# Aseeef/seq-align-gpu

Hardware: AMD Instinct MI355X
Metric: GCUPS (DP cell updates/s) at 1/2/4/8 MI355X; bit-exact max scores vs CPU ref (higher is better)
Workload: dtype f16

## Files before the change

seq-align-gpu_amd/__init__.py:

```python
import ctypes as C
import os

import numpy as np

_HERE = os.path.dirname(os.path.abspath(__file__))
LIB_PATH = os.path.join(_HERE, "libswg.so")
DATA_DIR = os.path.join(_HERE, "data")
CLI_PATH = os.path.join(_HERE, "bin", "smith_waterman")

if not os.path.exists(LIB_PATH):
    raise ImportError(
        "libswg.so is not built: run `python seq-align-gpu_amd/build.py` "
        "(or __graft_entry__.build()); there is no Python/CPU fallback")

lib = C.CDLL(LIB_PATH, mode=C.RTLD_GLOBAL)

SWG_OK, SWG_ERR_ARG, SWG_ERR_HIP, SWG_ERR_NOMEM = 0, -1, -2, -3
SWG_ERR_STATE, SWG_ERR_RESIDUE, SWG_ERR_IO, SWG_ERR_NODEVICE = -4, -5, -6, -7

ABI_SYMBOLS = [
    "swg_create", "swg_destroy", "swg_last_error", "swg_global_error", "swg_abi_version", "swg_prune_last",
    "swg_set_option", "swg_set_scoring", "swg_set_query", "swg_set_query_pssm", "swg_db_pack", "swg_db_pack_shard", "swg_db_pack_shards", "swg_db_upload", "swg_db_view",
    "swg_db_free", "swg_db_save", "swg_db_load", "swg_db_count", "swg_db_total_count", "swg_db_residues",
    "swg_db_packed_bytes", "swg_db_order", "swg_search", "swg_search_begin", "swg_search_end", "swg_search_multi",
# ... 187 lines not shown
_sig("swg_group_create", C.c_int, [_vp, C.c_int, C.c_int, C.POINTER(_vp)])
_sig("swg_group_destroy", None, [_vp])
_sig("swg_group_size", C.c_int, [_vp])
_sig("swg_group_last_error", C.c_char_p, [_vp])
_sig("swg_group_set_option", C.c_int, [_vp, C.c_char_p, C.c_long])
_sig("swg_group_set_scoring", C.c_int, [_vp, _vp, C.c_int, C.c_int])
_sig("swg_group_set_query", C.c_int, [_vp, _vp, C.c_size_t])
_sig("swg_group_set_query_pssm", C.c_int, [_vp, _vp, C.c_size_t])
_sig("swg_group_load", C.c_int, [_vp, _vp, _vp, C.c_size_t])
_sig("swg_group_search", C.c_int, [_vp, _vp, _vp, C.c_size_t, C.POINTER(C.c_size_t), C.POINTER(Stats)])
_sig("swg_letter_index", C.c_int, [C.c_int])
_sig("swg_index_letter", C.c_int, [C.c_int])
_sig("swg_scoring_init", None, [C.POINTER(Scoring)])
_sig("swg_scoring_add", C.c_int, [C.POINTER(Scoring), C.c_int, C.c_int, C.c_int])
_sig("swg_scoring_load_matrix", C.c_int, [C.POINTER(Scoring), C.c_char_p, C.c_char_p, C.c_size_t])
_sig("swg_query_sanitize", None, [C.POINTER(Scoring), _vp, C.c_size_t])
_sig("swg_seqs_read", C.c_int, [C.c_char_p, C.c_size_t, C.POINTER(Seqs), C.c_char_p, C.c_size_t])
_sig("swg_seqs_free", None, [C.POINTER(Seqs)])
_sig("swg_seqs_to_indices", C.c_int, [C.POINTER(Seqs), _vp, C.c_char_p])
_sig("swg_synth_db", C.c_int, [C.c_uint64, C.c_size_t, C.c_double, C.c_double, C.c_uint32,
                               C.c_uint32, C.POINTER(_vp), C.POINTER(_vp)])
_sig("swg_synth_query", None, [C.c_uint64, C.c_size_t, _vp])
_sig("swg_synth_db_similar", C.c_int, [C.c_uint64, C.c_size_t, C.c_double, C.c_double, C.c_uint32,
                                       C.c_uint32, _vp, C.c_size_t, C.c_double, C.c_double,
                                       C.POINTER(_vp), C.POINTER(_vp), C.POINTER(C.c_size_t)])
_sig("swg_synth_db_family", C.c_int, [C.c_uint64, C.c_size_t, C.c_double, C.c_double, C.c_uint32,
                                      C.c_uint32, _vp, C.c_size_t, C.c_double, C.c_double, C.c_double,
                                      C.POINTER(_vp), C.POINTER(_vp), C.POINTER(C.c_size_t)])
_sig("swg_synth_db_shard", C.c_int, [C.c_uint64, C.c_size_t, C.c_double, C.c_double, C.c_uint32, C.c_uint32,
                                     _vp, C.c_size_t, C.c_double, C.c_double, C.c_int, C.c_int,
                                     C.POINTER(_vp), C.POINTER(_vp), C.POINTER(_vp), C.POINTER(C.c_size_t),
                                     C.POINTER(C.c_uint64), C.POINTER(C.c_size_t)])
_sig("swg_synth_free", None, [_vp])
_sig("swg_pssm_load", C.c_int, [C.c_char_p, C.POINTER(Scoring), C.POINTER(_vp), C.POINTER(_vp), C.POINTER(C.c_size_t),
                                C.c_char_p, C.c_size_t])
_sig("swg_pssm_free", None, [_vp, _vp])
_sig("swg_debug_fail_alloc", None, [C.c_int])
_sig("swg_align_stats", C.c_int, [_vp, _vp, _vp, C.c_size_t, _vp, _vp])
_sig("swg_align_stats_multi", C.c_int, [_vp, _vp, _vp, _vp, C.c_size_t, _vp, C.c_size_t, _vp, _vp, _vp])
_sig("swg_align_stats_multi_pssm", C.c_int, [_vp, _vp, _vp, _vp, C.c_size_t, _vp, C.c_size_t, _vp, _vp, _vp])
_sig("swg_debug_bounds_last", C.c_int, [_vp, _vp])
_sig("swg_debug_sort_count", C.c_ulong, [])
_sig("swg_debug_engine", C.c_int, [_vp, C.c_size_t, C.c_int, C.c_int, _vp])
_sig("swg_debug_plan", C.c_int, [_vp, C.c_size_t, C.c_int, _vp])
_sig("swg_debug_plan_f16", C.c_int, [_vp, C.c_size_t, C.c_int, C.c_long, _vp])
_sig("swg_debug_plan_gapless", C.c_int, [_vp, C.c_size_t, C.c_int, _vp])
_sig("swg_debug_plan_forced", C.c_int, [_vp, C.c_size_t, C.c_int, C.c_long, C.c_long, C.c_long, C.c_int, C.c_long, C.c_int, _vp])
_sig("swg_debug_plan_streams", C.c_int, [_vp, _vp, _vp, C.c_size_t, C.c_int, C.c_long, C.c_long, C.c_long, C.c_long, _vp])
_sig("swg_debug_plan_systolic", C.c_int, [_vp, _vp, _vp, C.c_size_t, C.c_int, C.c_int, C.c_int, C.c_long, C.c_long, C.c_long, C.c_long, C.c_long, _vp])
_sig("swg_debug_systolic_variants", C.c_int, [C.c_int, _vp, C.c_size_t])
_sig("swg_debug_plan_batch", C.c_int, [_vp, C.c_size_t, C.c_size_t, C.c_int, C.c_int, C.c_int, C.c_long, C.c_long, C.c_long, _vp])
_sig("swg_debug_plan_lists", C.c_int, [_vp, C.c_size_t, C.c_size_t, C.c_int, C.c_int, C.c_long, C.c_long, C.c_long, _vp])
_sig("swg_debug_launch_log", None, [C.c_int])
_sig("swg_debug_launch_log_read", C.c_size_t, [_vp, C.c_size_t])
_sig("swg_debug_split", C.c_int, [_vp, C.c_size_t, C.c_uint64, _vp])
_sig("swg_debug_list_plan", C.c_int, [C.c_size_t, C.c_uint32, C.c_int, _vp, _vp])
_sig("swg_debug_pair_tokens", C.c_int, [_vp, _vp, C.c_int, _vp, C.c_size_t, C.POINTER(C.c_size_t)])
_sig("swg_debug_view_ranks", C.c_int, [_vp, _vp, C.c_size_t, _vp, C.POINTER(C.c_size_t)])
_sig("swg_debug_list_jobs", C.c_int, [_vp, _vp, _vp, C.c_size_t, _vp, C.c_size_t, C.POINTER(C.c_size_t), _vp])
_sig("swg_prune_last", C.c_int, [_vp, _vp])
_sig("swg_debug_prune_bound", C.c_int, [_vp, _vp, C.c_size_t, _vp, _vp, C.c_size_t, _vp, _vp])
_sig("swg_debug_prune_plan", C.c_int, [_vp, _vp])
_sig("swg_debug_prune_plan_above", C.c_int, [_vp, _vp])
_sig("swg_debug_above_multi_route", C.c_int, [C.c_long, C.c_int, C.c_int])
_sig("swg_debug_prune_stages", C.c_int, [_vp, _vp, C.c_size_t, C.POINTER(C.c_size_t)])
_sig("swg_debug_prune_kmer", C.c_int, [_vp, _vp, C.c_size_t, C.c_int, C.c_int, C.c_int, _vp, _vp, C.c_size_t, _vp, _vp])
_sig("swg_debug_prune_kmer_choice", C.c_int, [_vp, _vp])
_sig("swg_debug_prune_kmer_read", C.c_int, [_vp, _vp, C.c_int, _vp, _vp, C.c_size_t, _vp])
_sig("swg_debug_prune_kmer_seg", C.c_int, [_vp, _vp, C.c_size_t, C.c_int, C.c_int, C.c_int, C.c_int, _vp, _vp, C.c_size_t, _vp, _vp])
_sig("swg_debug_prune_kmer_choice_seg", C.c_int, [_vp, _vp])
_sig("swg_debug_prune_kmer_seg_read", C.c_int, [_vp, _vp, C.c_int, C.c_int, _vp, _vp, C.c_size_t, _vp])
_sig("swg_debug_prune_kmer_refine", C.c_int, [_vp, _vp, C.c_size_t, C.c_int, C.c_int, C.c_int, _vp, _vp, C.c_size_t, _vp, _vp])
_sig("swg_debug_prune_refine_choice", C.c_int, [_vp, _vp])
_sig("swg_debug_prune_refine_read", C.c_int, [_vp, _vp, C.c_int, _vp, _vp, _vp, C.c_size_t, _vp, C.c_size_t, _vp])
_sig("swg_debug_prune_stages3", C.c_int, [_vp, _vp, C.c_size_t, C.POINTER(C.c_size_t)])
_sig("swg_debug_prune_kmer_refine3", C.c_int, [_vp, _vp, C.c_size_t, C.c_int, C.c_int, C.c_int, _vp, _vp, C.c_size_t, _vp, _vp])
_sig("swg_debug_prune_refine3_choice", C.c_int, [_vp, _vp])
_sig("swg_debug_prune_kmer_refine4", C.c_int, [_vp, _vp, C.c_size_t, C.c_int, C.c_int, C.c_int, _vp, _vp, C.c_size_t, _vp])
_sig("swg_debug_prune_table_bits", C.c_int, [_vp, _vp, C.c_size_t, C.c_int])
_sig("swg_debug_prune_tables", C.c_int, [_vp, _vp])
_sig("swg_debug_prune_tables4", C.c_int, [_vp, _vp])
_sig("swg_debug_prune_refine4_read", C.c_int, [_vp, _vp, C.c_size_t, _vp])
_sig("swg_debug_prune_refine4_choice", C.c_int, [_vp, _vp])
_sig("swg_debug_prune_stages4", C.c_int, [_vp, _vp, C.c_size_t, C.POINTER(C.c_size_t)])
_sig("swg_debug_list_deal", C.c_int, [_vp, _vp, _vp, C.c_size_t, C.c_uint64, C.c_uint64, _vp, C.c_size_t, C.POINTER(C.c_size_t)])
_sig("swg_debug_calib_iters", C.c_int, [_vp, _vp, C.c_size_t, C.POINTER(C.c_size_t)])
_sig("swg_db_composition", C.c_int, [_vp, _vp, _vp])
_sig("swg_calibrate", C.c_int, [_vp, _vp, C.c_int, _vp])
_sig("swg_calibrate_multi", C.c_int, [_vp, _vp, _vp, C.c_size_t, _vp, C.c_int, _vp])
_sig("swg_calibrate_multi_pssm", C.c_int, [_vp, _vp, _vp, C.c_size_t, _vp, C.c_int, _vp])
_sig("swg_evalue", C.c_double, [_vp, C.c_uint64, C.c_int32])
_sig("swg_bitscore", C.c_double, [_vp, C.c_int32])
_sig("swg_evalue_min_score", C.c_int32, [_vp, C.c_uint64, C.c_double])
_sig("swg_synth_db_iid", C.c_int, [C.c_uint64, C.c_size_t, C.c_uint32, _vp, C.POINTER(_vp), C.POINTER(_vp)])
_sig("swg_gumbel_fit_hist", C.c_int, [_vp, C.c_size_t, C.POINTER(C.c_double), C.POINTER(C.c_double), C.POINTER(C.c_int)])
_sig("swg_matrix_lambda", C.c_int, [_vp, _vp, C.POINTER(C.c_double)])
_sig("swg_pssm_from_paths", C.c_int, [_vp, _vp, C.c_double, _vp, C.c_size_t, _vp, _vp, _vp, _vp, C.c_size_t, C.c_size_t, _vp, _vp, _vp])
_sig("swg_pssm_save", C.c_int, [C.c_char_p, _vp, _vp, C.c_size_t])
_sig("swg_pssm_build", C.c_int, [_vp, _vp, _vp, C.c_size_t, _vp, _vp, C.c_double, _vp, _vp, _vp])
_sig("swg_pssm_build_multi", C.c_int, [_vp, _vp, _vp, _vp, C.c_size_t, _vp, C.c_size_t, _vp, _vp, C.c_double, _vp, _vp, _vp])
_sig("swg_pssm_build_multi_pssm", C.c_int, [_vp, _vp, _vp, _vp, _vp, C.c_size_t, _vp, C.c_size_t, _vp, _vp, C.c_double, _vp, _vp, _vp])
_sig("swg_mask_params_default", None, [_vp])
_sig("swg_mask_tables", C.c_int, [_vp, _vp, C.POINTER(C.c_int64), C.POINTER(C.c_int64)])
_sig("swg_seg_mask", C.c_int, [_vp, C.c_size_t, _vp, _vp, C.POINTER(C.c_size_t)])
_sig("swg_seg_mask_segments", C.c_int, [_vp, C.c_size_t, _vp, _vp, C.POINTER(C.c_size_t), C.POINTER(C.c_size_t)])
_sig("swg_seg_mask_flat", C.c_int, [_vp, _vp, C.c_size_t, _vp, _vp])
_sig("swg_db_sequence", C.c_int, [_vp, C.c_uint32, _vp, C.c_size_t, C.POINTER(C.c_size_t)])
_sig("swg_db_mask", C.c_int, [_vp, _vp, _vp, C.POINTER(_vp)])
_sig("swg_db_mask_info", C.c_int, [_vp, _vp])
_sig("swg_debug_mask_fail_alloc", None, [C.c_int])


def _check(rc, ctx=None):
    if rc != SWG_OK:
        msg = lib.swg_last_error(ctx) if ctx else lib.swg_global_error()
        raise SwgError(rc, (msg or b"").decode("utf-8", "replace"))


def _i8(a):
    a = np.ascontiguousarray(a, dtype=np.int8)
    return a, a.ctypes.data_as(_vp)


def _pssm(pssm):
    a = np.asarray(pssm)
    if a.ndim != 2 or a.shape[1] != 32:
        raise ValueError("a PSSM is an (lq, 32) array, got shape %s" % (a.shape,))
    if a.dtype != np.int8 and a.size and (a.min() < -128 or a.max() > 127):
        raise ValueError("PSSM values must fit int8")
    p, pp = _i8(a)
    return p, pp, a.shape[0]


def _lists(lists):
    arrs = [np.ascontiguousarray(l, dtype=np.uint32).reshape(-1) for l in lists]
    off = np.zeros(len(arrs) + 1, dtype=np.uint64)
    off[1:] = np.cumsum([a.size for a in arrs])
    flat = np.concatenate(arrs) if arrs else np.zeros(0, dtype=np.uint32)
    if flat.size == 0:
        flat = np.zeros(1, dtype=np.uint32)
    return np.ascontiguousarray(flat, dtype=np.uint32), off


def letters_to_indices(s):
    out = np.empty(len(s), dtype=np.int8)
    for i, ch in enumerate(s):
        v = lib.swg_letter_index(ord(ch))
        if v < 0:
            raise SwgError(SWG_ERR_RESIDUE, "illegal residue %r" % ch)
        out[i] = v
    return out


def load_scoring(name_or_path, gap_open=-2, gap_extend=-1):
    path = name_or_path
    if not os.path.exists(path):
        path = os.path.join(DATA_DIR, name_or_path + ".txt")
    sc = Scoring()
    lib.swg_scoring_init(C.byref(sc))
    err = C.create_string_buffer(512)
    rc = lib.swg_scoring_load_matrix(C.byref(sc), path.encode(), err, 512)
    if rc != SWG_OK:
        raise SwgError(rc, err.value.decode())
    sc.gap_open, sc.gap_extend = gap_open, gap_extend
    return sc

# ... 242 lines not shown
    a = np.array([forced, pruned, lq, pair_rows, table_rate, fill_rate], dtype=np.int64)
    out = np.zeros(1, dtype=np.int64)
    _check(lib.swg_debug_prune_kmer_choice(a.ctypes.data_as(_vp), out.ctypes.data_as(_vp)))
    return int(out[0])


KMER_MAX_SEGMENTS = 32
KMER_TABLE_BUDGET = 96 << 20


def debug_prune_kmer_seg(rows, query, gap_open, gap_extend, k, segments, flat, offsets, table=True):
    S = int(segments)
    return _prune_kmer_mirror(lib.swg_debug_prune_kmer_seg, rows, query, gap_open, gap_extend, (int(k), S), flat, offsets,
                              (KMER_CLASSES ** int(k), S) if table and k in (4, 5) and 1 <= S <= KMER_MAX_SEGMENTS else None)


def debug_prune_kmer_choice_seg(forced=0, segments=0, pruned=1, lq=3000, pair_rows=1900000000, table_rate=0, fill_rate=0):
    a = np.array([forced, pruned, lq, pair_rows, table_rate, fill_rate, segments], dtype=np.int64)
    out = np.zeros(4, dtype=np.int64)
    _check(lib.swg_debug_prune_kmer_choice_seg(a.ctypes.data_as(_vp), out.ctypes.data_as(_vp)))
    return int(out[0]), int(out[1]), int(out[2]), bool(out[3])


KMER_REFINE_SEGMENTS = 128
KMER_REFINE3_SEGMENTS = 256


def debug_prune_kmer_refine(rows, query, gap_open, gap_extend, segments, flat, offsets, table=True):
    S = int(segments)
    hook = lib.swg_debug_prune_kmer_refine3 if S == KMER_REFINE3_SEGMENTS else lib.swg_debug_prune_kmer_refine
    return _prune_kmer_mirror(hook, rows, query, gap_open, gap_extend, (S,), flat, offsets,
                              (KMER_CLASSES ** 4, S) if table and S in (32, 64, 128, 256) else None)


def debug_prune_kmer_refine4(rows, query, gap_open, gap_extend, segments, flat, offsets):
    r, rp = _i8(rows)
    lq = r.size // 32
    qp = None
    if query is not None:
        q, qp = _i8(query)
        lq = q.size
    f, fp = _i8(flat)
    off = np.ascontiguousarray(offsets, dtype=np.uint64)
    n = off.size - 1
    u = np.zeros(max(n, 1), dtype=np.uint64)
    _check(lib.swg_debug_prune_kmer_refine4(rp, qp, lq, int(gap_open), int(gap_extend), int(segments), fp, off.ctypes.data_as(_vp), n,
                                            u.ctypes.data_as(_vp)))
    return u[:n]


def debug_prune_table_bits(rows, query, k=4):
    r, rp = _i8(rows)
    lq = r.size // 32
    qp = None
    if query is not None:
        q, qp = _i8(query)
        lq = q.size
    rc = lib.swg_debug_prune_table_bits(rp, qp, lq, int(k))
    if rc < 0:
        _check(rc)
    return rc


def debug_prune_refine3_choice(forced=0, segments=0, refine=0, refine3=0, table_bits=8, pruned=1, lq=3000, pair_rows=1900000000,
                               table_rate=0, fill_rate=0):
    a = np.array([forced, pruned, lq, pair_rows, table_rate, fill_rate, segments, refine, refine3, table_bits], dtype=np.int64)
    out = np.zeros(4, dtype=np.int64)
    _check(lib.swg_debug_prune_refine3_choice(a.ctypes.data_as(_vp), out.ctypes.data_as(_vp)))
    return int(out[0]), int(out[1]), int(out[2]), int(out[3])


KMER_REFINE4_SEGMENTS = 256
PRUNE_REFINE4_FORCED = 5256


def debug_prune_refine4_choice(forced=0, segments=0, refine=0, refine3=0, refine4=0, table_bits=8, table_bits5=8, pruned=1, lq=3000,
                               pair_rows=1900000000, table_rate=0, fill_rate=0):
    a = np.array([forced, pruned, lq, pair_rows, table_rate, fill_rate, segments, refine, refine3, table_bits, refine4, table_bits5], dtype=np.int64)
    out = np.zeros(5, dtype=np.int64)
    _check(lib.swg_debug_prune_refine4_choice(a.ctypes.data_as(_vp), out.ctypes.data_as(_vp)))
    return tuple(int(v) for v in out)


def debug_prune_refine_choice(forced=0, segments=0, refine=0, pruned=1, lq=3000, pair_rows=1900000000, table_rate=0, fill_rate=0):
    a = np.array([forced, pruned, lq, pair_rows, table_rate, fill_rate, segments, refine], dtype=np.int64)
    out = np.zeros(3, dtype=np.int64)
    _check(lib.swg_debug_prune_refine_choice(a.ctypes.data_as(_vp), out.ctypes.data_as(_vp)))
    return int(out[0]), int(out[1]), int(out[2])


def prune_list(bounds, begin, end, threshold):
    b = np.asarray(bounds)[begin:end]
    return (begin + np.nonzero(b >= threshold)[0]).astype(np.uint32)


PRUNE_PLAN_KEYS = ("mode", "k", "want_scores", "gap_open", "gap_extend", "bits", "use_diag", "n_classes", "work_queue", "both_forms",
                   "gapless", "batch", "range_pairs", "groups", "prune_head", "n_segments")


def debug_prune_plan(**ask):
    d = dict(mode=1, k=100, want_scores=0, gap_open=-2, gap_extend=-1, bits=16, use_diag=1, n_classes=1, work_queue=1, both_forms=0,
             gapless=0, batch=0, range_pairs=1000000, groups=1024, prune_head=4, n_segments=8)
    unknown = set(ask) - set(d)
    if unknown:
        raise TypeError("debug_prune_plan: unknown arguments %s" % sorted(unknown))
    d.update(ask)
    a = np.array([int(d[k]) for k in PRUNE_PLAN_KEYS], dtype=np.int64)
    out = np.zeros(2, dtype=np.int64)
    _check(lib.swg_debug_prune_plan(a.ctypes.data_as(_vp), out.ctypes.data_as(_vp)))
    return bool(out[0]), int(out[1])


PRUNE_PLAN_ABOVE_KEYS = ("mode", "gap_open", "gap_extend", "bits", "use_diag", "n_classes", "work_queue", "both_forms", "gapless", "batch",
                         "range_pairs", "groups", "n_segments", "prune_head")


def debug_prune_plan_above(**ask):
    d = dict(mode=1, gap_open=-2, gap_extend=-1, bits=16, use_diag=1, n_classes=1, work_queue=1, both_forms=0, gapless=0, batch=0,
             range_pairs=1000000, groups=1024, n_segments=8, prune_head=4)
    unknown = set(ask) - set(d)
    if unknown:
        raise TypeError("debug_prune_plan_above: unknown arguments %s" % sorted(unknown))
    d.update(ask)
    a = np.array([int(d[k]) for k in PRUNE_PLAN_ABOVE_KEYS], dtype=np.int64)
    out = np.zeros(2, dtype=np.int64)
    _check(lib.swg_debug_prune_plan_above(a.ctypes.data_as(_vp), out.ctypes.data_as(_vp)))
    return bool(out[0]), int(out[1])


def debug_above_multi_route(option=0, admitted=True, single_pruned=False):
    rc = lib.swg_debug_above_multi_route(int(option), 1 if admitted else 0, 1 if single_pruned else 0)
    if rc < 0:
        _check(rc)
    return rc


PRUNE_STAGE_QUEUED = ("threshold", "prefix_cut", "gate", "refine", "list")
_PRUNE_STAGE_BITS = ((0, "threshold"), (1, "prefix_cut"), (2, "gate"), (3, "refine"), (5, "refine3"), (6, "refine4"), (4, "list"))


def debug_prune_stages(segments, head_pairs=0, fixed=False, refine=0, prefix_cut=False, refine3=0, refine4=0):
    a = np.array([head_pairs, fixed, refine, prefix_cut, refine3, refine4, len(segments)] + [int(v) for sg in segments for v in sg], dtype=np.int64)
    out = np.zeros((2 * len(segments) + 1, 4), dtype=np.int64)
    n = C.c_size_t(0)
    _check(lib.swg_debug_prune_stages4(a.ctypes.data_as(_vp), out.ctypes.data_as(_vp), out.shape[0], C.byref(n)))
    return [(int(b), int(e), int(sg), tuple(name for i, name in _PRUNE_STAGE_BITS if int(qd) >> i & 1))
            for b, e, sg, qd in out[:n.value]]


LAUNCH_FAMILIES = ("dyn", "lists", "q32", "qq", "streams", "systolic")


def debug_systolic_variants(bits):
    out = np.zeros((16, 2), dtype=np.int32)
    n = lib.swg_debug_systolic_variants(bits, out.ctypes.data_as(_vp), 16)
    assert 0 < n <= 16
    return [(int(k), int(w)) for k, w in out[:n]]


def debug_launch_log(on):
    lib.swg_debug_launch_log(1 if on else 0)


def debug_launch_log_read():
    seen = lib.swg_debug_launch_log_read(None, 0)
    out = np.zeros((max(seen, 1), 10), dtype=np.int32)
    lib.swg_debug_launch_log_read(out.ctypes.data_as(_vp), seen)
    kept = int(np.count_nonzero(out[:seen, 1]))
    if kept < seen:
        raise SwgError(SWG_ERR_STATE, "launch log: %d launches, %d kept" % (seen, kept))
    keys = ("family", "K", "G", "W", "form", "edges", "flag", "workgroups", "grid_rows", "list")
    recs = []
    for row in out[:seen]:
        r = dict(zip(keys, (int(v) for v in row)))
        r["family"] = LAUNCH_FAMILIES[r["family"]]
        r["fma"] = r["exact"] = r.pop("flag")
        recs.append(r)
    return recs


def synth_query(seed, lq):
    out = np.empty(lq, dtype=np.int8)
    lib.swg_synth_query(seed, lq, out.ctypes.data_as(_vp))
    return out


def hit_key(score, index):
    return int(lib.swg_hit_key(int(score), int(index)))


def key_hit(key):
    h = Hit()
    lib.swg_key_hit(int(key), C.byref(h))
    return int(h.score), int(h.index)


def topk_merge_keys(keys, k):
    keys = np.ascontiguousarray(keys, dtype=np.uint64)
    out = (Hit * max(k, 1))()
    m = lib.swg_topk_merge_keys(keys.ctypes.data_as(_vp), keys.size, k, C.cast(out, _vp))
    return [(int(out[i].score), int(out[i].index)) for i in range(m)]


def mask_params(window=12, trigger=2.2, extend=2.5, replace=MASK_REPLACE_DEFAULT):
    return MaskParams(int(window), int(replace), float(trigger), float(extend))


def mask_tables(window=12, trigger=2.2, extend=2.5, replace=MASK_REPLACE_DEFAULT):
    p = mask_params(window, trigger, extend, replace)
    T = np.zeros(65, dtype=np.int32)
    t1, t2 = C.c_int64(0), C.c_int64(0)
    _check(lib.swg_mask_tables(C.byref(p), T.ctypes.data_as(_vp), C.byref(t1), C.byref(t2)))
    return T, t1.value, t2.value


def seg_mask(seq, window=12, trigger=2.2, extend=2.5, replace=MASK_REPLACE_DEFAULT, want_segments=False):
    a, ap = _i8(seq)
    p = mask_params(window, trigger, extend, replace)
    m = np.zeros(max(1, a.size), dtype=np.uint8)
    nm, ns = C.c_size_t(0), C.c_size_t(0)
    _check(lib.swg_seg_mask_segments(ap, a.size, C.byref(p), m.ctypes.data_as(_vp), C.byref(nm), C.byref(ns)))
    mask = m[:a.size].astype(bool)
    assert int(mask.sum()) == nm.value
    return (mask, ns.value) if want_segments else mask


def debug_mask_fail_alloc(n):
    lib.swg_debug_mask_fail_alloc(int(n))
# ... 571 lines not shown
        qoff[1:] = np.cumsum([len(q) for q in queries])
        qflat = np.ascontiguousarray(np.concatenate(queries) if len(queries) else np.zeros(0), dtype=np.int8)
        return self._align_multi(lib.swg_align_stats_multi, db, qflat, qoff, hits, False, None, bounds=True, stats=True)

    def align_stats_multi_pssm(self, db, pssms, hits):
        rows = [_pssm(p)[0] for p in pssms]
        qoff = np.zeros(len(rows) + 1, dtype=np.uint64)
        qoff[1:] = np.cumsum([r.shape[0] for r in rows])
        pflat = np.ascontiguousarray(np.concatenate(rows) if rows else np.zeros((0, 32)), dtype=np.int8)
        return self._align_multi(lib.swg_align_stats_multi_pssm, db, pflat, qoff, hits, False, None, bounds=True, stats=True)

    @staticmethod
    def _stats_dict(al, cnt):
        a = {f: int(getattr(al, f)) for f, _ in Alignment._fields_ if f != "reserved"}
        a.update((f, int(getattr(cnt, f))) for f, _ in AlignCounts._fields_)
        return a

    def prune_last(self):

        class _Info(C.Structure):
            _fields_ = [("pairs_skipped", C.c_uint64), ("pair_rows_skipped", C.c_uint64), ("pair_rows", C.c_uint64),
                        ("threshold", C.c_uint32), ("pruned", C.c_int32)]

        i = _Info()
        _check(lib.swg_prune_last(self.handle, C.cast(C.byref(i), _vp)), self.handle)
        return {"pruned": bool(i.pruned), "threshold": int(i.threshold), "pairs_skipped": int(i.pairs_skipped),
                "pair_rows_skipped": int(i.pair_rows_skipped), "pair_rows": int(i.pair_rows)}

    def debug_prune_kmer_read(self, db, k=None, bounds=False):
        info = np.zeros(3, dtype=np.uint64)
        t = np.zeros(KMER_CLASSES ** int(k), dtype=np.uint16) if k else None
        n = 0
        if bounds:
            _check(lib.swg_debug_prune_kmer_read(self.handle, db.handle, 0, None, None, 0, info.ctypes.data_as(_vp)), self.handle)
            n = int(info[2])
        b = np.zeros(max(n, 1), dtype=np.uint32) if bounds else None
        _check(lib.swg_debug_prune_kmer_read(self.handle, db.handle, int(k or 0), t.ctypes.data_as(_vp) if t is not None else None,
                                             b.ctypes.data_as(_vp) if b is not None else None, n, info.ctypes.data_as(_vp)), self.handle)
        return {"k": int(info[0]), "builds": int(info[1]), "pairs": int(info[2]), "table": t, "bounds": None if b is None else b[:int(info[2])]}

    def debug_prune_kmer_seg_read(self, db, k=None, segments=1, bounds=False):
        info = np.zeros(4, dtype=np.uint64)
        S = int(segments)
        t = np.zeros((KMER_CLASSES ** int(k), S), dtype=np.uint16) if k else None
        n = 0
        if bounds:
            _check(lib.swg_debug_prune_kmer_seg_read(self.handle, db.handle, 0, 0, None, None, 0, info.ctypes.data_as(_vp)), self.handle)
            n = int(info[2])
        b = np.zeros(max(n, 1), dtype=np.uint32) if bounds else None
        _check(lib.swg_debug_prune_kmer_seg_read(self.handle, db.handle, int(k or 0), S, t.ctypes.data_as(_vp) if t is not None else None,
                                                 b.ctypes.data_as(_vp) if b is not None else None, n, info.ctypes.data_as(_vp)), self.handle)
        return {"k": int(info[0]), "builds": int(info[1]), "pairs": int(info[2]), "segments": int(info[3]), "table": t,
                "bounds": None if b is None else b[:int(info[2])]}

    def debug_prune_refine_read(self, db, segments=None, arrays=True):
        info = np.zeros(7, dtype=np.uint64)
        _check(lib.swg_debug_prune_refine_read(self.handle, db.handle, 0, None, None, None, 0, None, 0, info.ctypes.data_as(_vp)), self.handle)
        n = int(info[2])
        if not arrays:
            return {"k": int(info[0]), "builds": int(info[1]), "pairs": n, "segments": int(info[3]), "refine": int(info[4]),
                    "refine_builds": int(info[5]), "table": None, "bounds": None, "stages": []}
        S = int(segments or 0)
        t = np.zeros((KMER_CLASSES ** 4, S), dtype=np.uint16) if S else None
        b = np.zeros(max(n, 1), dtype=np.uint32)
        l = np.zeros(max(n, 1), dtype=np.uint32)
        st = np.zeros((256, 4), dtype=np.uint32)
        _check(lib.swg_debug_prune_refine_read(self.handle, db.handle, S, t.ctypes.data_as(_vp) if t is not None else None, b.ctypes.data_as(_vp),
                                               l.ctypes.data_as(_vp), n, st.ctypes.data_as(_vp), 256, info.ctypes.data_as(_vp)), self.handle)
        stages = [(int(r[0]), int(r[1]), int(r[2]), l[int(r[0]):int(r[0]) + int(r[3])].copy()) for r in st[:int(info[6])]]
        return {"k": int(info[0]), "builds": int(info[1]), "pairs": n, "segments": int(info[3]), "refine": int(info[4]),
                "refine_builds": int(info[5]), "table": t, "bounds": b[:n], "stages": stages}

    def debug_prune_tables(self):
        out = np.zeros(7, dtype=np.int64)
        _check(lib.swg_debug_prune_tables(self.handle, out.ctypes.data_as(_vp)), self.handle)
        return {"refine3": int(out[0]), "refine3_builds": int(out[1]),
                "bits": dict(zip(("first4", "first5", "second", "third"), (int(v) for v in out[2:6]))), "auto_bits": int(out[6])}

    def debug_prune_tables4(self):
        out = np.zeros(4, dtype=np.int64)
        _check(lib.swg_debug_prune_tables4(self.handle, out.ctypes.data_as(_vp)), self.handle)
        return {"refine4": int(out[0]), "refine4_builds": int(out[1]), "bits": int(out[2]), "refused": bool(out[3])}

    def debug_prune_refine4_read(self, blocks):
        b = np.ascontiguousarray(blocks, dtype=np.uint32)
        out = np.zeros((max(b.size, 1), KMER_REFINE4_SEGMENTS), dtype=np.uint16)
        _check(lib.swg_debug_prune_refine4_read(self.handle, b.ctypes.data_as(_vp), b.size, out.ctypes.data_as(_vp)), self.handle)
        return out[:b.size]

    def debug_bounds_last(self):
        out = np.zeros(4, dtype=np.uint32)
        _check(lib.swg_debug_bounds_last(self.handle, out.ctypes.data_as(_vp)), self.handle)
        return dict(zip(("kernel_pairs", "fallback_pairs", "launches", "column_limit"), (int(v) for v in out)))

    def _align_multi(self, fn, db, qflat, qoff, hits, want_ops, ops_stride, bounds=False, stats=False):
        nq = len(qoff) - 1
        if len(hits) != nq:
            raise ValueError("hits: %d rows for %d queries" % (len(hits), nq))
        k = max((len(row) for row in hits), default=0)
        arr = (Hit * max(nq * k, 1))()
        nh = (C.c_size_t * max(nq, 1))()
        for i, row in enumerate(hits):
            nh[i] = len(row)
            for j, (sc, ix) in enumerate(row):
                arr[i * k + j].score, arr[i * k + j].index = int(sc), int(ix)
        out = (Alignment * max(nq * k, 1))()
        stride = 0 if bounds else int(ops_stride if ops_stride is not None else
                                      lib.swg_align_ops_bound_multi(db.handle, qoff.ctypes.data_as(_vp), nq))
        ops = C.create_string_buffer(max(1, nq * k * stride)) if want_ops else None
        args = (self.handle, db.handle, qflat.ctypes.data_as(_vp), qoff.ctypes.data_as(_vp), nq, C.cast(arr, _vp), k,
                C.cast(nh, _vp), C.cast(out, _vp))
        if stats:
            cnt = (AlignCounts * max(nq * k, 1))()
            _check(fn(*args, C.cast(cnt, _vp)), self.handle)
            return [[self._stats_dict(out[i * k + j], cnt[i * k + j]) for j in range(len(row))] for i, row in enumerate(hits)]
        _check(fn(*args) if bounds else fn(*args, C.cast(ops, _vp) if want_ops else None, stride), self.handle)
        raw = ops.raw if want_ops else None
        res = []
        for i, row in enumerate(hits):
            r = []
            for j in range(len(row)):
                h = i * k + j
                a = {f: int(getattr(out[h], f)) for f, _ in Alignment._fields_ if f != "reserved"}
                if want_ops:
                    a["ops"] = raw[h * stride:h * stride + a["n_ops"]].decode()
                r.append(a)
            res.append(r)
        return res

    @staticmethod
    def _hit_keys(hits, k, n):
        a = np.frombuffer(hits, dtype=np.dtype([("score", "<i4"), ("index", "<u4")]), count=max(k, 1))[:k]
        keys = (a["score"].astype(np.uint64) << np.uint64(32)) | (np.uint64(0xFFFFFFFF) - a["index"].astype(np.uint64))
        keys[n:] = 0
        return keys

    def search_keys(self, db, k):
        hits = (Hit * max(k, 1))()
        nh = C.c_size_t(0)
        st = Stats()
        _check(lib.swg_search(self.handle, db.handle, None, C.cast(hits, _vp), k, C.byref(nh), C.byref(st)),
               self.handle)
        a = np.frombuffer(hits, dtype=np.dtype([("score", "<i4"), ("index", "<u4")]), count=max(k, 1))[:k]
        keys = (a["score"].astype(np.uint64) << np.uint64(32)) | (np.uint64(0xFFFFFFFF) - a["index"].astype(np.uint64))
        keys[nh.value:] = 0
        return keys, st.as_dict()

    def fill_batches16(self, batches):
        arr = (Batch16 * len(batches))()
        keep, outs = [], []
        for i, (d, vs) in enumerate(batches):
            d = np.ascontiguousarray(d, dtype=np.int8)
            o = np.zeros(16, dtype=np.int16)
            keep.append(d)
            outs.append(o)
            arr[i].db_idx_t = d.ctypes.data
            arr[i].max_len = d.shape[0]
            arr[i].vector_size = vs
            arr[i].max_scores = o.ctypes.data
        secs = C.c_double(0)
        _check(lib.swg_fill_batches16(self.handle, arr, len(batches), C.byref(secs)), self.handle)
        return [o[:vs].copy() for o, (_, vs) in zip(outs, batches)], secs.value

    def close(self):
        if self.handle:
            lib.swg_destroy(self.handle)
# ... 83 lines not shown
```

seq-align-gpu_amd/csrc/swg_api.cpp:

```cpp
#include "swg_host_internal.h"
#include "../../include/swg_host.h"

#include <algorithm>
#include <atomic>
#include <chrono>
#include <climits>
#include <cmath>
#include <cstdarg>
#include <cstdio>
#include <cstdlib>
#include <cstring>
#include <new>
#include <vector>

static thread_local std::string g_err;
static std::atomic<uint64_t> g_epoch{1};

int swg_set_global_error(int code, const char *fmt, ...)
{
    char buf[512];
    va_list ap;
    va_start(ap, fmt);
    vsnprintf(buf, sizeof buf, fmt, ap);
    va_end(ap);
// ... 225 lines not shown

extern "C" int swg_set_option(swg_ctx *ctx, const char *key, long value)
{
    if (!ctx || !key) return swg_set_ctx_error(ctx, SWG_ERR_ARG, "swg_set_option: NULL argument");
    if (!strcmp(key, "force_bits")) {
        if (value != 0 && value != 16 && value != 32)
            return swg_set_ctx_error(ctx, SWG_ERR_ARG, "force_bits must be 0, 16 or 32");
        ctx->opt_force_bits = value;
    } else if (!strcmp(key, "cols_per_wave")) {
        ctx->opt_cols = value;
    } else if (!strcmp(key, "max_waves")) {
        if (value < 0 || value > 16) return swg_set_ctx_error(ctx, SWG_ERR_ARG, "max_waves must be 0..16");
        ctx->opt_max_waves = value;
    } else if (!strcmp(key, "engine")) {
        if (value < 0 || value > 2) return swg_set_ctx_error(ctx, SWG_ERR_ARG, "engine must be 0 (auto), 1 (systolic) or 2 (diagonal)");
        ctx->opt_engine = value;
    } else if (!strcmp(key, "group_lanes")) {
        if (value != 0 && value != 16 && value != 32 && value != 64)
            return swg_set_ctx_error(ctx, SWG_ERR_ARG, "group_lanes must be 0, 16, 32 or 64");
        ctx->opt_group = value;
    } else if (!strcmp(key, "long_cols")) {
        extern long g_swg_long_cols;
        g_swg_long_cols = value;
    } else if (!strcmp(key, "long_group")) {
        extern long g_swg_long_group;
        g_swg_long_group = value;
    } else if (!strcmp(key, "autotune")) {
        ctx->opt_autotune = value != 0;
    } else if (!strcmp(key, "side_readout")) {
        ctx->opt_side_readout = value != 0;
    } else if (!strcmp(key, "wide16")) {
        ctx->opt_wide = value != 0;
    } else if (!strcmp(key, "f16")) {
        if (value < 0 || value > 2) return swg_set_ctx_error(ctx, SWG_ERR_ARG, "f16 must be 0 (off), 1 (auto) or 2 (whenever the gap scores allow)");
        ctx->opt_f16 = value;
    } else if (!strcmp(key, "f16_pair")) {
        if (value < 0 || value > 2)
            return swg_set_ctx_error(ctx, SWG_ERR_ARG, "f16_pair must be 0 (auto), 1 (v_perm_b32) or 2 (v_pk_fma_f16 wherever it fits)");
        ctx->opt_f16_pair = value;
    } else if (!strcmp(key, "bounds_groups")) {
        if (value < 0) return swg_set_ctx_error(ctx, SWG_ERR_ARG, "bounds_groups must be 0 (auto) or the most lane groups of a bounds launch");
        ctx->opt_bounds_groups = value;
    } else if (!strcmp(key, "last_pass")) {
        ctx->opt_last_pass = value != 0;
    } else if (!strcmp(key, "qq")) {
        ctx->opt_qq = value != 0;
    } else if (!strcmp(key, "batch_geometry")) {
        if (value != 0 && value != 1)
            return swg_set_ctx_error(ctx, SWG_ERR_ARG, "batch_geometry must be 0 (a forced geometry sends a batch one by one) or 1 (the batch takes it)");
        ctx->opt_batch_geometry = value;
    } else if (!strcmp(key, "long_helps")) {
        ctx->opt_long_helps = value != 0;
    } else if (!strcmp(key, "segment_blocks")) {
        if (value < 0 || value > (long)SWG_DYN_SEG_BLOCKS)
            return swg_set_ctx_error(ctx, SWG_ERR_ARG, "segment_blocks must be 0 (default) .. 2^26-64");
        ctx->opt_seg_blocks = value ? (uint32_t)value : SWG_DYN_SEG_BLOCKS;
    } else if (!strcmp(key, "prune")) {
        if (value < 0 || value > 2)
            return swg_set_ctx_error(ctx, SWG_ERR_ARG, "prune must be 0 (off), 1 (auto) or 2 (wherever it is structurally possible: diagnostic)");
        ctx->opt_prune = value;
    } else if (!strcmp(key, "prune_head")) {
        if (value < 0 || value > 4096) return swg_set_ctx_error(ctx, SWG_ERR_ARG, "prune_head must be 0..4096 (pairs per lane group)");
        ctx->opt_prune_head = value;
    } else if (!strcmp(key, "prune_kmer")) {
        if (value != 0 && value != 1 && value != 4 && value != 5)
            return swg_set_ctx_error(ctx, SWG_ERR_ARG, "prune_kmer must be 0 (auto), 1 (the colmax bound), 4 or 5 (the k-mer bound of that k)");
        ctx->opt_prune_kmer = value;
    } else if (!strcmp(key, "prune_segments")) {
        if (value < 0 || value > (long)SWG_KMER_MAX_SEGMENTS)
            return swg_set_ctx_error(ctx, SWG_ERR_ARG, "prune_segments must be 0 (auto) or 1..32 (the segments of the k-mer bound's table; 1: unsegmented)");
        ctx->opt_prune_segments = value;
    } else if (!strcmp(key, "prune_refine")) {
        if (!swg_prune_refine_value_ok(value))
            return swg_set_ctx_error(ctx, SWG_ERR_ARG, "prune_refine must be 0 (auto), 1 (off), 64 or 128 (the segments of the second-level bound's table)");
        ctx->opt_prune_refine = value;
    } else if (!strcmp(key, "prune_refine3")) {
        if (!swg_prune_refine3_value_ok(value))
            return swg_set_ctx_error(ctx, SWG_ERR_ARG, "prune_refine3 must be 0 (auto), 1 (off) or 256 (the segments of the third-level bound's table)");
        ctx->opt_prune_refine3 = value;
    } else if (!strcmp(key, "prune_refine4")) {
        if (!swg_prune_refine4_value_ok(value))
            return swg_set_ctx_error(ctx, SWG_ERR_ARG, "prune_refine4 must be 0 (auto), 1 (off) or 5256 (the fourth-level bound's table: k = 5 in 256 segments)");
        ctx->opt_prune_refine4 = value;
    } else if (!strcmp(key, "prune_table_bits")) {
        if (value != 0 && value != 16)
            return swg_set_ctx_error(ctx, SWG_ERR_ARG, "prune_table_bits must be 0 (auto: bytes where they hold every entry) or 16");
        ctx->opt_prune_table_bits = value;
    } else if (!strcmp(key, "prune_cut")) {
        if (value != 0 && value != 1)
            return swg_set_ctx_error(ctx, SWG_ERR_ARG, "prune_cut must be 0 (a stage's pairs are cut one by one) or 1 (the prefix of the length order)");
        ctx->opt_prune_cut = value;
    } else if (!strcmp(key, "above_batch")) {
        if (value < 0 || value > 2)
            return swg_set_ctx_error(ctx, SWG_ERR_ARG, "above_batch must be 0 (auto), 1 (one launch wherever the batch is admitted) or 2 (one query after another)");
        ctx->opt_above_batch = value;
    } else if (!strcmp(key, "calib_seqs")) {
        if (value < 2 || value > (1l << 20)) return swg_set_ctx_error(ctx, SWG_ERR_ARG, "calib_seqs must be 2..1048576 (random sequences a calibration scores)");
        ctx->opt_calib_seqs = value;
    } else if (!strcmp(key, "pssm_msa_mb")) {
        if (value < 0 || value > 65536) return swg_set_ctx_error(ctx, SWG_ERR_ARG, "pssm_msa_mb must be 0..65536 (MiB of device rows one group of queries of swg_pssm_build* may take; 0: every query alone)");
        ctx->opt_pssm_msa_mb = value;
    } else if (!strcmp(key, "calib_len")) {
        if (value < 8 || value > (1l << 14)) return swg_set_ctx_error(ctx, SWG_ERR_ARG, "calib_len must be 8..16384 (residues of a calibration's random sequences)");
        ctx->opt_calib_len = value;
    } else if (!strcmp(key, "calib_seed")) {
        if (value < 0) return swg_set_ctx_error(ctx, SWG_ERR_ARG, "calib_seed must be >= 0");
        ctx->opt_calib_seed = value;
    } else if (!strcmp(key, "q32_waves")) {
        ctx->opt_q32_waves = value;
    } else if (!strcmp(key, "wave_budget")) {
        ctx->opt_wave_budget = value;
    } else if (!strcmp(key, "batch")) {
        if (value < 0 || value > 8) return swg_set_ctx_error(ctx, SWG_ERR_ARG, "batch must be 0..8 (pairs one queue request claims; 0 and 1: one)");
        ctx->opt_batch = value;
    } else if (!strcmp(key, "batch_blocks")) {
        if (value < 0) return swg_set_ctx_error(ctx, SWG_ERR_ARG, "batch_blocks must be >= 0 (token blocks; 0: from the geometry)");
        ctx->opt_batch_blocks = value;
    } else if (!strcmp(key, "work_queue")) {
        ctx->opt_dynamic = value != 0;
    } else if (!strcmp(key, "prio_share")) {
        if (value < 0) return swg_set_ctx_error(ctx, SWG_ERR_ARG, "prio_share must be >= 0 (percent)");
        ctx->opt_prio_share = value;
    } else if (!strcmp(key, "long_split")) {
        if (value < -1) return swg_set_ctx_error(ctx, SWG_ERR_ARG, "long_split must be -1 (off), 0 (auto) or a row count");
        ctx->opt_long_split = value;
    } else if (!strcmp(key, "workgroups")) {
        if (value < 0) return swg_set_ctx_error(ctx, SWG_ERR_ARG, "workgroups must be >= 0");
        ctx->opt_workgroups = value;
    } else {
        return swg_set_ctx_error(ctx, SWG_ERR_ARG, "swg_set_option: unknown key '%s'", key);
    }
    return SWG_OK;
}

extern "C" int swg_set_scoring(swg_ctx *ctx, const int8_t sub[32][32], int gap_open, int gap_extend)
{
    if (!ctx || !sub) return swg_set_ctx_error(ctx, SWG_ERR_ARG, "swg_set_scoring: NULL argument");
    if (gap_open < -32768 || gap_open > 32767 || gap_extend < -32768 || gap_extend > 32767)
        return swg_set_ctx_error(ctx, SWG_ERR_ARG,
                                 "swg_set_scoring: gap scores must fit the reference's int16 score_t");
    HIP_TRY(ctx, hipSetDevice(ctx->device));
    memcpy(ctx->sub, sub, 32 * 32);
    ctx->gap_open = gap_open;
    ctx->gap_extend = gap_extend;
    HIP_TRY(ctx, hipMemcpyAsync(ctx->d_sub, ctx->sub, 32 * 32, hipMemcpyHostToDevice, ctx->stream));
    HIP_TRY(ctx, hipStreamSynchronize(ctx->stream));
    ctx->have_scoring = true;
    ctx->epoch = g_epoch.fetch_add(1) + 1;
    return SWG_OK;
}

static int stage_query(swg_ctx *ctx, int8_t *dst, const int8_t *src, size_t bytes)
{
    const int b = ctx->query_stage_next;
    ctx->query_stage_next = (b + 1) % 4;
    if (!ctx->ev_query_stage[b]) HIP_TRY(ctx, hipEventCreateWithFlags(&ctx->ev_query_stage[b], hipEventDisableTiming));
    else HIP_TRY(ctx, hipEventSynchronize(ctx->ev_query_stage[b]));
    if (bytes > ctx->h_query_stage_cap[b]) {
        (void)hipHostFree(ctx->h_query_stage[b]);
        ctx->h_query_stage[b] = nullptr;
        ctx->h_query_stage_cap[b] = 0;
        HIP_TRY(ctx, hipHostMalloc(reinterpret_cast<void **>(&ctx->h_query_stage[b]), bytes, hipHostMallocDefault));
        ctx->h_query_stage_cap[b] = bytes;
    }
    memcpy(ctx->h_query_stage[b], src, bytes);
    HIP_TRY(ctx, hipMemcpyAsync(dst, ctx->h_query_stage[b], bytes, hipMemcpyHostToDevice, ctx->stream));
// ... 632 lines not shown
    size_t slice = 0;
    std::vector<std::pair<uint32_t, uint32_t>> segs;
    bool first_launch = true;
    int launches = 0, f16_launches = 0;

    int launch(int pass, const std::pair<uint32_t, uint32_t> &sg, uint32_t b, uint32_t en, int pform, const uint8_t *prof, bool f16_part)
    {
        const SwgDiagPlan &pl = wk.plan[c];
        const SwgPairTokens &T = db->ptok;
        q.profile = prof + (size_t)pass * slice;
        q.edge_in = pass > 0 ? T.d_edge[(pass - 1) & 1] : nullptr;
        q.edge_out = pass + 1 < pl.npass ? T.d_edge[pass & 1] : nullptr;
        if (!first_launch)
            HIP_TRY(ctx, hipMemsetAsync(q.queue, 0, (size_t)SWG_DYN_SHARDS * SWG_DYN_SHARD_STRIDE * 4, qs));
        first_launch = false;
        q.q_begin = b;
        q.q_end = en;
        if (cut) {
            q.seg_origin = T.pair_blocks_prefix[sg.first];
            q.seg_blocks = T.pair_blocks_prefix[sg.second] - q.seg_origin;
        }
        const int variant = pass + 1 == pl.npass && pl.npass > 1 && pl.last_variant >= 0 ? pl.last_variant : pl.variant;
        const int wgs_c = diag_class_workgroups(ctx, db, wk, c);
        if (!(ctx->opt_long_helps && wk.n_classes == 2)) dyn_batch_zones(ctx, T, &q, (uint64_t)wgs_c * pl.W * (64 / pl.G), swg_diag_variant_info(variant).K, pl.G, pform);
        HIP_TRY(ctx, swg_launch_diag_dyn(variant, edges, pform, pl.W, wgs_c, q, qs, 1, fma));
        ++launches;
        if (f16_part) ++f16_launches;
        return SWG_OK;
    }
};

static int dyn_fill_begin(DynFill *F, int go, int ge, uint64_t *d_trace)
{
    swg_ctx *ctx = F->ctx;
    const swg_db *db = F->db;
    const SwgDiagWork &wk = F->wk;
    const int c = F->c;
    const SwgDiagPlan &pl = wk.plan[c];
    const SwgPairTokens &T = db->ptok;
    SwgDiagDynParams &q = F->q;
    F->form = diag_class_form(ctx, db, pl);
    q = dyn_params_base(T, db->d_scores, (size_t)db->n_bins * SWG_BIN, pl.G, F->form, go, ge, wk.n_classes, db->d_counters + SWG_RANK_WORD(c));
    q.q_begin = (uint32_t)wk.pair_begin[c];
    q.q_end = (uint32_t)wk.pair_end[c];
    q.queue = db->d_counters + SWG_QUEUE_WORD(c);
    q.profile = ctx->d_profile[diag_profile_slot(pl, c)];
    auto bulk_prio = [&]() -> uint32_t {
        const uint64_t blocks = T.pair_blocks_prefix[wk.pair_end[0]] - T.pair_blocks_prefix[wk.pair_begin[0]];
        return bulk_prio_blocks(ctx, blocks, (uint64_t)diag_class_workgroups(ctx, db, wk, 0) * wk.plan[0].W * (64 / wk.plan[0].G));
    };
    q.prio_blocks = c == 1 ? 0u : bulk_prio();
    if (c == 1 && ctx->opt_long_helps && diag_class_is_dynamic(ctx, db, wk.plan[0])) {
        q.q2_begin = (uint32_t)wk.pair_begin[0];
        q.q2_end = (uint32_t)wk.pair_end[0];
        q.queue2 = db->d_counters + SWG_QUEUE_WORD(0);
        q.prio_blocks2 = bulk_prio();
    }
    q.f16_wipe = ctx->cur->plan.score_bound >= 32000ull ? 1u : 0u;
    q.trace = d_trace;
    q.stamps = pl.npass == 1 ? reinterpret_cast<unsigned long long *>(db->d_counters + SWG_WORD_STAMPS(c)) : nullptr;
    F->edges = pl.npass > 1 || F->form == 1;
    F->fma = diag_class_fma(ctx, db, pl);
    F->slice = swg_diag_slice_bytes(pl.K, pl.G, F->fma);
    F->qs = c == 1 ? ctx->stream2 : ctx->stream;
    if (!token_segments(T, q.q_begin, q.q_end, ctx->opt_seg_blocks, F->edges, &F->segs, &F->cut))
        return swg_set_ctx_error(ctx, SWG_ERR_ARG, "a pair of sequences too long for the multi-pass fill");
    q.seg_origin = 0;
    q.seg_blocks = (uint32_t)std::min<uint64_t>(T.total_blocks, ctx->opt_seg_blocks);
    if (F->cut) {
        q.q2_begin = q.q2_end = 0;
        q.queue2 = nullptr;
    }
    return SWG_OK;
}

static int enqueue_pruned_fill(swg_ctx *ctx, swg_db *db, const SwgPrunePlan &pr, size_t k, DynFill *F)
{
    const SwgPairTokens &T = db->ptok;
    const SwgDiagPlan &pl = F->wk.plan[F->c];
    hipStream_t qs = F->qs;
    uint32_t *thr = db->d_counters + SWG_PRUNE_WORD_T, *cut_word = db->d_counters + SWG_PRUNE_WORD_CUT, *gate = db->d_counters + SWG_PRUNE_WORD_GATE;
    const uint32_t n_pairs = (uint32_t)swg_db_pair_count(db);
    const SwgPruneLayout L = swg_prune_layout(db->d_pair_bound, n_pairs);
    if (pr.kmer > 1 && pr.segments > 1)
        HIP_TRY(ctx, swg_launch_pair_bound_kmer_seg(T.d_tok, T.d_pair_off, n_pairs, pr.kmer, (uint32_t)pr.segments, ctx->prune_colmax, ctx->kmer_first[pr.kmer - 4].d,
                                                    ctx->kmer_first[pr.kmer - 4].bits, L.bounds, L.ids, qs));
    else if (pr.kmer > 1)
        HIP_TRY(ctx, swg_launch_pair_bound_kmer(T.d_tok, T.d_pair_off, n_pairs, pr.kmer, ctx->prune_colmax, ctx->kmer_first[pr.kmer - 4].d,
                                                ctx->kmer_first[pr.kmer - 4].bits, L.bounds, L.ids, qs));
    else
        HIP_TRY(ctx, swg_launch_pair_bound(T.d_tok, T.d_pair_off, n_pairs, ctx->prune_colmax, L.bounds, L.ids, qs));
    if (pr.fixed) HIP_TRY(ctx, hipMemsetD32Async(reinterpret_cast<hipDeviceptr_t>(thr), (int)pr.fixed_T, 1, qs));
    db->prune_stages.clear();
    for (const SwgPruneStage &st : swg_prune_stages(pr, F->segs)) {
        if (st.queued & SWG_STAGE_THRESHOLD)
            HIP_TRY(ctx, swg_launch_prune_threshold(db->d_scores, db->d_order, (uint32_t)((size_t)db->n_bins * SWG_BIN), (uint32_t)k, db->d_hist, thr, qs));
        if (st.queued & SWG_STAGE_PREFIX_CUT) HIP_TRY(ctx, swg_launch_prune_cut(L.bounds, T.d_pair_off, st.begin, st.end, thr, cut_word, qs));
        if (st.queued & SWG_STAGE_GATE) HIP_TRY(ctx, swg_launch_prune_refine_gate(L.bounds, st.begin, st.end, thr, gate, qs));
        if (st.queued & SWG_STAGE_REFINE)
            HIP_TRY(ctx, swg_launch_pair_bound_refine(T.d_tok, T.d_pair_off, st.begin, st.end, (uint32_t)pr.refine, ctx->prune_colmax, ctx->kmer_second.d,
                                                      ctx->kmer_second.bits, st.queued & SWG_STAGE_GATE ? gate : thr, L.bounds, qs));
        if (st.queued & SWG_STAGE_REFINE3)
            HIP_TRY(ctx, swg_launch_pair_bound_refine(T.d_tok, T.d_pair_off, st.begin, st.end, (uint32_t)pr.refine3, ctx->prune_colmax, ctx->kmer_third.d,
                                                      ctx->kmer_third.bits, st.queued & SWG_STAGE_GATE ? gate : thr, L.bounds, qs));
        if (st.queued & SWG_STAGE_REFINE4)
            HIP_TRY(ctx, swg_launch_pair_bound_refine(T.d_tok, T.d_pair_off, st.begin, st.end, (uint32_t)pr.refine4, ctx->prune_colmax, ctx->kmer_fourth.d,
                                                      ctx->kmer_fourth.bits, st.queued & SWG_STAGE_GATE ? gate : thr, L.bounds, qs, 5));
        if (st.queued & SWG_STAGE_LIST) {
            const size_t rec = db->prune_stages.size() / 2;
            HIP_TRY(ctx, swg_launch_prune_list(L.bounds, T.d_pair_off, st.begin, st.end, thr, L.tiles, L.lists + st.begin, cut_word,
                                               rec < SWG_PRUNE_STAGE_RECS ? L.recs + 2 * rec : nullptr, qs));
            db->prune_stages.push_back(st.begin), db->prune_stages.push_back(st.end);
        }
        F->q.list = st.queued & SWG_STAGE_PREFIX_CUT ? L.ids + st.begin : st.queued & SWG_STAGE_LIST ? L.lists + st.begin : nullptr;
        F->q.list_count = F->q.list ? cut_word : nullptr;
        for (int pass = 0; pass < pl.npass; ++pass) {
            const int rc = F->launch(pass, F->segs[st.segment], st.begin, st.end, F->form, ctx->d_profile[diag_profile_slot(pl, F->c)], false);
            if (rc != SWG_OK) return rc;
        }
    }
    F->q.list = nullptr, F->q.list_count = nullptr;
    return SWG_OK;
}

static int launch_diag(swg_ctx *ctx, swg_db *db, const SwgDiagWork &wk, int go, int ge, bool *two_ends,
                       const SwgPrunePlan *prune = nullptr, size_t prune_k = 0)
{
    hipStream_t s = ctx->stream;
    *two_ends = false;
    static const char *trace_path = getenv("SWG_TRACE");
    uint64_t *d_trace[2] = {nullptr, nullptr};
    if (trace_path)
        for (int c = 0; c < wk.n_classes; ++c) {
            const size_t bytes = (size_t)wk.plan[c].workgroups * wk.plan[c].W * 4 * 8;
            HIP_TRY(ctx, hipMalloc(&d_trace[c], bytes));
            HIP_TRY(ctx, hipMemsetAsync(d_trace[c], 0, bytes, s));
        }
    HIP_TRY(ctx, hipEventRecord(ctx->cur->ev[1], s));
    int rf = fork_long_class(ctx, wk);
    if (rf != SWG_OK) return rf;
    for (int c = wk.n_classes - 1; c >= 0; --c) {
        const SwgDiagLayout &L = db->diag[c];
        const SwgDiagPlan &pl = wk.plan[c];
        if (diag_class_is_dynamic(ctx, db, pl)) {
            DynFill F{ctx, db, wk, c};
            int rc = dyn_fill_begin(&F, go, ge, d_trace[c]);
            if (rc != SWG_OK) return rc;
            const uint32_t class_begin = F.q.q_begin, class_end = F.q.q_end;
            const bool split = c == 0 && wk.n_classes == 1 && F.form != 2 && pl.f16_from > class_begin && pl.f16_from < class_end;
            const bool pruned = prune && prune->on && c == 0 && wk.n_classes == 1 && !split && db->d_pair_bound;
            if (c == 0) ctx->cur->pruned = pruned;
            if (pruned) {
                if ((rc = enqueue_pruned_fill(ctx, db, *prune, prune_k, &F)) != SWG_OK) return rc;
            } else
            for (int part = 0; part < (split ? 2 : 1); ++part) {
                const int pform = split && part == 1 ? 2 : F.form;
                const uint32_t part_begin = split && part == 1 ? pl.f16_from : class_begin;
                const uint32_t part_end = split && part == 0 ? pl.f16_from : class_end;
                const uint8_t *prof = ctx->d_profile[split && part == 1 ? 7 : diag_profile_slot(pl, c)];
                F.q.go = gap_word(pform, go);
                F.q.ge = gap_word(pform, ge);
                if (split && part == 1) HIP_TRY(ctx, hipEventRecord(ctx->cur->ev[5], F.qs));
                for (int pass = 0; pass < pl.npass; ++pass) {
                    for (const std::pair<uint32_t, uint32_t> &sg : F.segs) {
                        const uint32_t b = std::max(sg.first, part_begin), en = std::min(sg.second, part_end);
                        if (b >= en) continue;
                        if ((rc = F.launch(pass, sg, b, en, pform, prof, split && part == 1)) != SWG_OK) return rc;
                    }
                }
            }
            if (c == 0) ctx->cur->fill_launches = F.launches, ctx->cur->fill_f16_launches = F.f16_launches;
            continue;
        }
        SwgDiagParams d;
        memset(&d, 0, sizeof d);
        d.tok = L.d_tok;
        d.stream_off = L.d_stream_off;
        d.stream_pairs = L.d_stream_pairs;
        d.stream_pair_off = L.d_stream_pair_off;
// ... 774 lines not shown
    if (rescore && !systolic_plan(32, (uint32_t)std::min<size_t>(n_slots / 64, 1u << 30), 0, max_waves, workgroups, lq, n_cu, &re)) return SWG_OK;
    const int32_t v[12] = {1, pl.K, pl.W, pl.npass, pl.workgroups, takes_f16 ? 1 : 0, pl.info.max_waves, bits, rescore ? 1 : 0, re.K, re.W, re.npass};
    memcpy(out, v, sizeof v);
    return SWG_OK;
}
extern "C" int swg_debug_systolic_variants(int bits, int32_t *out, size_t cap)
{
    if (bits != 16 && bits != 32) return 0;
    const int n = swg_num_variants(bits);
    for (int v = 0; out && v < n && (size_t)v < cap; ++v) {
        const SwgKernelInfo info = swg_variant_info(bits, v);
        out[2 * v] = info.K, out[2 * v + 1] = info.max_waves;
    }
    return n;
}

static void ensure_prune_colmax(swg_ctx *ctx)
{
    if (ctx->prune_colmax_epoch == ctx->epoch) return;
    ctx->prune_colmax = ctx->query_pssm ? swg_prune_colmax(ctx->pssm.data(), nullptr, ctx->query_len())
                                        : swg_prune_colmax(&ctx->sub[0][0], ctx->query.data(), ctx->query_len());
    ctx->prune_colmax_epoch = ctx->epoch;
}
static int kmer_table_bits(swg_ctx *ctx, int k)
{
    ensure_prune_colmax(ctx);
    return ctx->opt_prune_table_bits == 16 ? 16 : swg_kmer_table_bits(ctx->prune_colmax, k);
}

static int plan_prune(swg_ctx *ctx, swg_db *db, bool want_scores, size_t k, SwgSearchPlan *P)
{
    P->prune = SwgPrunePlan();
    if (!P->use_diag || P->bits != 16) return SWG_OK;
    const SwgDiagWork &wk = P->wk;
    const SwgDiagPlan &pl = wk.plan[0];
    SwgPruneAsk a;
    a.mode = (int)ctx->opt_prune;
    a.k = k;
    a.want_scores = want_scores;
    a.gap_open = ctx->gap_open;
    a.gap_extend = ctx->gap_extend;
    a.bits = P->bits;
    a.use_diag = P->use_diag;
    a.n_classes = wk.n_classes;
    a.work_queue = diag_class_is_dynamic(ctx, db, pl) && db->ptok.ok;
    a.both_forms = P->split_at != 0u;
    a.gapless = P->gapless;
    a.batch = ctx->in_batch;
    a.prune_head = ctx->opt_prune_head;
    a.fixed = ctx->above_min > 0;
    if (a.mode == 0 || !a.work_queue || wk.n_classes != 1) return SWG_OK;
    a.range_pairs = wk.pair_end[0] - wk.pair_begin[0];
    a.groups = diag_class_streams(ctx, db, wk, 0);
    const int form = diag_class_form(ctx, db, pl);
    std::vector<std::pair<uint32_t, uint32_t>> segs;
    bool cut = false;
    if (!token_segments(db->ptok, (uint32_t)wk.pair_begin[0], (uint32_t)wk.pair_end[0], ctx->opt_seg_blocks, pl.npass > 1 || form == 1, &segs, &cut))
        return SWG_OK;
    a.n_segments = segs.size();
    P->prune = swg_prune_plan(a);
    ctx->prune_choice = SwgPruneChoice();
    if (!P->prune.on) return SWG_OK;
    P->prune.fixed_T = P->prune.fixed ? (uint32_t)ctx->above_min : 0u;
    SwgKmerAsk ka;
    ka.forced = ctx->opt_prune_kmer;
    ka.forced_segments = ctx->opt_prune_segments;
    ka.forced_refine = ctx->opt_prune_refine;
    ka.forced_refine3 = ctx->opt_prune_refine3;
    ka.forced_refine4 = ctx->opt_prune_refine4;
    ensure_prune_colmax(ctx);
    ka.table_bits = kmer_table_bits(ctx, 4);
    ka.table_bits5 = kmer_table_bits(ctx, 5);
    ka.pruned = true;
    ka.lq = ctx->query_len();
    ka.pair_rows = 4ull * (db->ptok.pair_blocks_prefix[wk.pair_end[0]] - db->ptok.pair_blocks_prefix[wk.pair_begin[0]]);
    ka.fill_rate = swg_kmer_fill_rate(ka.lq);
    P->prune.kmer = swg_prune_kmer_choice(ka, &P->prune.segments);
    P->prune.prefix_cut = ctx->opt_prune_cut == 1 && !P->prune.fixed;
    P->prune.refine = P->prune.prefix_cut ? 0 : swg_prune_refine_choice(ka, P->prune.kmer, P->prune.segments);
    P->prune.refine3 = P->prune.prefix_cut ? 0 : swg_prune_refine3_choice(ka, P->prune.kmer, P->prune.segments, P->prune.refine);
    P->prune.refine4 = P->prune.prefix_cut || ctx->kmer_fourth_refused
                           ? 0
                           : swg_prune_refine4_choice(ka, P->prune.kmer, P->prune.segments, P->prune.refine, P->prune.refine3);
    ctx->prune_choice = SwgPruneChoice{P->prune.kmer, P->prune.segments, P->prune.refine, P->prune.refine3, P->prune.refine4};
    return SWG_OK;
}

static int ensure_kmer_table(swg_ctx *ctx, SwgKmerTable *t, int k, int S)
{
    const int bits = kmer_table_bits(ctx, k);
    if (t->holds(ctx->epoch, k, S, bits)) return SWG_OK;
    const size_t lq = ctx->query_len();
    int rc;
    if ((rc = device_grow(ctx, &ctx->d_kmer_cprof, &ctx->d_kmer_cprof_cap, lq * 32)) != SWG_OK) return rc;
    const size_t bytes = (size_t)swg_kmer_entries(k) * (size_t)S * (size_t)(bits / 8);
    if (t->cap < bytes) t->epoch = 0;
    if ((rc = device_grow(ctx, &t->d, &t->cap, bytes)) != SWG_OK) return rc;
    const long go = (long)ctx->gap_open + ctx->gap_extend, ge = ctx->gap_extend;
    HIP_TRY(ctx, swg_launch_kmer_table(ctx->d_sub, ctx->d_query, ctx->query_pssm ? ctx->d_pssm : nullptr, (uint32_t)lq, (uint32_t)-go, (uint32_t)-ge, k,
                                       (uint32_t)S, ctx->d_kmer_cprof, t->d, bits, ctx->stream));
    t->epoch = ctx->epoch, t->k = k, t->segments = S, t->bits = bits;
    ++(t == &ctx->kmer_fourth  ? ctx->kmer_refine4_builds
       : t == &ctx->kmer_third ? ctx->kmer_refine3_builds
       : t == &ctx->kmer_second ? ctx->kmer_refine_builds
                                : ctx->kmer_builds);
    return SWG_OK;
}

static bool reserve_kmer_fourth(swg_ctx *ctx)
{
    SwgKmerTable *t = &ctx->kmer_fourth;
    const size_t bytes = (size_t)swg_kmer_entries(5) * SWG_KMER_REFINE4_SEGMENTS;
    if (t->d && t->cap >= bytes) return true;
    (void)hipFree(t->d);
    t->d = nullptr, t->cap = 0, t->epoch = 0;
    uint8_t *d = nullptr;
    if (hipSetDevice(ctx->device) != hipSuccess || hipMalloc(&d, bytes) != hipSuccess) {
        (void)hipGetLastError();
        ctx->kmer_fourth_refused = true;
        return false;
    }
    t->d = d, t->cap = bytes;
    return true;
}

static int prepare_prune(swg_ctx *ctx, swg_db *db, const SwgPrunePlan &pr)
{
    int rc;
    ensure_prune_colmax(ctx);
    if (pr.kmer > 1) {
        const int k = pr.kmer, S = pr.segments;
        if (S < 1 || S > (int)SWG_KMER_MAX_SEGMENTS) return swg_set_ctx_error(ctx, SWG_ERR_ARG, "the k-mer bound's table: %d segments (1..32)", S);
        if (!swg_kmer_table_admitted(k, S))
            return swg_set_ctx_error(ctx, SWG_ERR_ARG, "the k-mer bound's table of k = %d in %d segments is %zu MB: above its budget of %zu MB (prune_kmer, prune_segments)", k,
                                     S, (size_t)swg_kmer_entries(k) * (size_t)S * sizeof(uint16_t) >> 20, (size_t)(SWG_KMER_TABLE_BUDGET >> 20));
        if ((rc = ensure_kmer_table(ctx, &ctx->kmer_first[k - 4], k, S)) != SWG_OK) return rc;
    }
    if (pr.refine) {
        if (pr.refine != 64 && pr.refine != 128) return swg_set_ctx_error(ctx, SWG_ERR_ARG, "the second-level bound's table: %d segments (64 or 128)", pr.refine);
        if ((rc = ensure_kmer_table(ctx, &ctx->kmer_second, 4, pr.refine)) != SWG_OK) return rc;
    }
    if (pr.refine3) {
        if (pr.refine3 != 256) return swg_set_ctx_error(ctx, SWG_ERR_ARG, "the third-level bound's table: %d segments (256)", pr.refine3);
        if ((rc = ensure_kmer_table(ctx, &ctx->kmer_third, 4, pr.refine3)) != SWG_OK) return rc;
    }
    if (pr.refine4) {
        if (pr.refine4 != (int)SWG_KMER_REFINE4_SEGMENTS || !swg_kmer_refine4_admitted(kmer_table_bits(ctx, 5)))
            return swg_set_ctx_error(ctx, SWG_ERR_ARG, "the fourth-level bound's table: %d segments (256) of bytes", pr.refine4);
        if ((rc = ensure_kmer_table(ctx, &ctx->kmer_fourth, 5, pr.refine4)) != SWG_OK) return rc;
    }
    swg_db::Bufs &b = db->bufs[ctx->cur - ctx->slots];
    const size_t n_pairs = (size_t)swg_db_pair_count(db);
    if ((rc = device_grow(ctx, &b.d_pair_bound, &b.pair_bound_cap, n_pairs, swg_prune_layout(b.d_pair_bound, n_pairs).words - n_pairs)) != SWG_OK) return rc;
    db->d_pair_bound = b.d_pair_bound;
    return SWG_OK;
}

static int prepare_search(swg_ctx *ctx, swg_db *db, const SwgSearchPlan &P)
{
    int rc = SWG_OK;
    const bool systolic_fill = !P.use_diag && !P.use_q32 && !(P.bits == 32 && P.use_diag32);
    const bool systolic_rescore = P.may_saturate && !P.use_diag32;
    const size_t bin32_scratch = P.bin32 && P.npass32 > 1 ? ((size_t)db->max_nblk * 4 + 4) * 4 * 16 * (size_t)ctx->n_cu : 0;
    if (P.bin32) {
        rc = ensure_profile_cols(ctx, 1, (uint32_t)(P.npass32 * 64 * SWG_DIAG32_K), 4, (1ull << 30) ^ (uint64_t)P.npass32);
        if (rc != SWG_OK) return rc;
        if ((rc = ensure_scratch(ctx, bin32_scratch)) != SWG_OK) return rc;
// ... 398 lines not shown
    st.topk_ms = topk_dev_ms + std::chrono::duration<double, std::milli>(std::chrono::steady_clock::now() - t0).count();
    if (stats) *stats = st;
    return SWG_OK;
}

static int debug_prune_read(swg_ctx *ctx, const swg_db *db, const char *fn, const SwgKmerTable *table, int k, int S, uint16_t *table_out, uint32_t *bound_out,
                            uint32_t *list_out, size_t pair_cap, uint32_t *stages_out, size_t stages_cap, int n_info, uint64_t *info)
{
    if (!ctx || !info) return swg_set_ctx_error(ctx, SWG_ERR_ARG, "%s: NULL argument", fn);
    HIP_TRY(ctx, hipSetDevice(ctx->device));
    HIP_TRY(ctx, hipDeviceSynchronize());
    const size_t n_pairs = db ? (size_t)swg_db_pair_count(db) : 0;
    const uint64_t all[7] = {(uint64_t)ctx->prune_choice.kmer, ctx->kmer_builds, n_pairs, (uint64_t)ctx->prune_choice.segments, (uint64_t)ctx->prune_choice.refine,
                             ctx->kmer_refine_builds, 0};
    std::copy(all, all + n_info, info);
    if (table_out) {
        if (!table || !table->holds(ctx->epoch, k, S, table->bits))
            return swg_set_ctx_error(ctx, SWG_ERR_STATE, "%s: no table of k = %d in %d segments for the current query and scoring", fn, k, S);
        const size_t entries = (size_t)swg_kmer_entries(k) * (size_t)S;
        if (table->bits == 8) {
            std::vector<uint8_t> narrow(entries);
            HIP_TRY(ctx, hipMemcpy(narrow.data(), table->d, entries, hipMemcpyDeviceToHost));
            std::copy(narrow.begin(), narrow.end(), table_out);
        } else
            HIP_TRY(ctx, hipMemcpy(table_out, table->d, entries * sizeof(uint16_t), hipMemcpyDeviceToHost));
    }
    if (bound_out || list_out || stages_out) {
        if (!db || !db->d_pair_bound || pair_cap < n_pairs) return swg_set_ctx_error(ctx, SWG_ERR_STATE, "%s: no pair bounds on this database, or too little room", fn);
        const SwgPruneLayout L = swg_prune_layout(db->d_pair_bound, n_pairs);
        if (bound_out) HIP_TRY(ctx, hipMemcpy(bound_out, L.bounds, n_pairs * sizeof(uint32_t), hipMemcpyDeviceToHost));
        if (list_out) HIP_TRY(ctx, hipMemcpy(list_out, L.lists, n_pairs * sizeof(uint32_t), hipMemcpyDeviceToHost));
        if (stages_out) {
            const size_t n = std::min<size_t>(std::min<size_t>(db->prune_stages.size() / 2, SWG_PRUNE_STAGE_RECS), stages_cap);
            std::vector<uint32_t> recs(2 * n);
            if (n) HIP_TRY(ctx, hipMemcpy(recs.data(), L.recs, 2 * n * sizeof(uint32_t), hipMemcpyDeviceToHost));
            for (size_t i = 0; i < n; ++i)
                stages_out[4 * i] = db->prune_stages[2 * i], stages_out[4 * i + 1] = db->prune_stages[2 * i + 1], stages_out[4 * i + 2] = recs[2 * i],
                               stages_out[4 * i + 3] = recs[2 * i + 1];
            info[6] = n;
        }
    }
    return SWG_OK;
}
extern "C" int swg_debug_prune_kmer_read(swg_ctx *ctx, const swg_db *db, int k, uint16_t *table_out, uint32_t *bound_out, size_t bound_cap,
                                         uint64_t *info)
{
    return debug_prune_read(ctx, db, "swg_debug_prune_kmer_read", ctx && (k == 4 || k == 5) ? &ctx->kmer_first[k - 4] : nullptr, k, 1, table_out, bound_out, nullptr,
                            bound_cap, nullptr, 0, 3, info);
}
extern "C" int swg_debug_prune_kmer_seg_read(swg_ctx *ctx, const swg_db *db, int k, int S, uint16_t *table_out, uint32_t *bound_out, size_t bound_cap,
                                             uint64_t *info)
{
    return debug_prune_read(ctx, db, "swg_debug_prune_kmer_seg_read", ctx && (k == 4 || k == 5) ? &ctx->kmer_first[k - 4] : nullptr, k, S, table_out, bound_out, nullptr,
                            bound_cap, nullptr, 0, 4, info);
}
extern "C" int swg_debug_prune_refine_read(swg_ctx *ctx, const swg_db *db, int S2, uint16_t *table_out, uint32_t *bound_out, uint32_t *list_out, size_t pair_cap,
                                           uint32_t *stages_out, size_t stages_cap, uint64_t *info)
{
    return debug_prune_read(ctx, db, "swg_debug_prune_refine_read", ctx ? (S2 == 256 ? &ctx->kmer_third : &ctx->kmer_second) : nullptr, 4, S2, table_out, bound_out,
                            list_out, pair_cap, stages_out, stages_cap, 7, info);
}
extern "C" int swg_debug_prune_tables(swg_ctx *ctx, int64_t *out)
{
    if (!ctx || !out) return swg_set_ctx_error(ctx, SWG_ERR_ARG, "swg_debug_prune_tables: NULL argument");
    const SwgKmerTable *t[4] = {&ctx->kmer_first[0], &ctx->kmer_first[1], &ctx->kmer_second, &ctx->kmer_third};
    out[0] = ctx->prune_choice.refine3;
    out[1] = (int64_t)ctx->kmer_refine3_builds;
    for (int i = 0; i < 4; ++i) out[2 + i] = t[i]->d && t[i]->epoch == ctx->epoch ? t[i]->bits : 0;
    out[6] = 0;
    if (ctx->query_len() > 0) {
        ensure_prune_colmax(ctx);
        out[6] = swg_kmer_table_bits(ctx->prune_colmax, 4);
    }
    return SWG_OK;
}

extern "C" int swg_debug_prune_tables4(swg_ctx *ctx, int64_t *out)
{
    if (!ctx || !out) return swg_set_ctx_error(ctx, SWG_ERR_ARG, "swg_debug_prune_tables4: NULL argument");
    out[0] = ctx->prune_choice.refine4;
    out[1] = (int64_t)ctx->kmer_refine4_builds;
    out[2] = ctx->kmer_fourth.d && ctx->kmer_fourth.epoch == ctx->epoch ? ctx->kmer_fourth.bits : 0;
    out[3] = ctx->kmer_fourth_refused ? 1 : 0;
    return SWG_OK;
}
extern "C" int swg_debug_prune_refine4_read(swg_ctx *ctx, const uint32_t *blocks, size_t n, uint16_t *out)
{
    if (!ctx || (n > 0 && (!blocks || !out))) return swg_set_ctx_error(ctx, SWG_ERR_ARG, "swg_debug_prune_refine4_read: NULL argument");
    const SwgKmerTable &t = ctx->kmer_fourth;
    HIP_TRY(ctx, hipSetDevice(ctx->device));
    HIP_TRY(ctx, hipDeviceSynchronize());
    if (!t.holds(ctx->epoch, 5, (int)SWG_KMER_REFINE4_SEGMENTS, 8))
        return swg_set_ctx_error(ctx, SWG_ERR_STATE, "swg_debug_prune_refine4_read: no fourth-level table for the current query and scoring");
    uint8_t row[SWG_KMER_REFINE4_SEGMENTS];
    for (size_t i = 0; i < n; ++i) {
        if (blocks[i] >= swg_kmer_entries(5)) return swg_set_ctx_error(ctx, SWG_ERR_ARG, "swg_debug_prune_refine4_read: block %u", blocks[i]);
        HIP_TRY(ctx, hipMemcpy(row, t.d + (size_t)blocks[i] * SWG_KMER_REFINE4_SEGMENTS, sizeof row, hipMemcpyDeviceToHost));
        std::copy(row, row + SWG_KMER_REFINE4_SEGMENTS, out + i * SWG_KMER_REFINE4_SEGMENTS);
    }
    return SWG_OK;
}

extern "C" int swg_prune_last(const swg_ctx *ctx, swg_prune_info *out)
{
    if (!ctx || !out) return SWG_ERR_ARG;
    *out = ctx->prune_last;
    return SWG_OK;
}

static int search_begin_ticket(swg_ctx *ctx, swg_db *db, bool want_scores, size_t k, bool allow_autotune, int *ticket)
{
    return ctx_guarded(ctx, "swg_search_begin", [&]() -> int {
        fail_alloc_here(1);
        if (!ctx || !db || !ticket) return swg_set_ctx_error(ctx, SWG_ERR_ARG, "swg_search_begin: NULL argument");
        int slot = -1;
        for (int i = 0; i < SWG_MAX_INFLIGHT; ++i) {
            const int c = (ctx->next_slot + i) % SWG_MAX_INFLIGHT;
            if (!ctx->slots[c].busy) {
                slot = c;
                break;
            }
        }
        if (slot < 0)
            return swg_set_ctx_error(ctx, SWG_ERR_STATE, "swg_search_begin: %d searches already in flight", SWG_MAX_INFLIGHT);
        const int rc = search_begin(ctx, db, want_scores, k, allow_autotune, &ctx->slots[slot]);
        if (rc != SWG_OK) return rc;
        ctx->slots[slot].busy = true;
        ctx->next_slot = (slot + 1) % SWG_MAX_INFLIGHT;
        *ticket = slot;
        return SWG_OK;
    });
}

extern "C" int swg_search_begin(swg_ctx *ctx, const swg_db *db, int want_scores, size_t k, int *ticket)
{
    return search_begin_ticket(ctx, const_cast<swg_db *>(db), want_scores != 0, k, ctx && ctx->opt_autotune != 0, ticket);
}

extern "C" int swg_search_end(swg_ctx *ctx, int ticket, int32_t *scores_out, swg_hit *topk_out, size_t *n_hits,
                              swg_stats *stats)
{
    bool valid = false;
    const int rc = ctx_guarded(ctx, "swg_search_end", [&]() -> int {
        fail_alloc_here(2);
        if (!ctx || ticket < 0 || ticket >= SWG_MAX_INFLIGHT || !ctx->slots[ticket].busy)
            return swg_set_ctx_error(ctx, SWG_ERR_ARG, "swg_search_end: no search in flight under that ticket");
        valid = true;
        return search_end(ctx, &ctx->slots[ticket], scores_out, topk_out, n_hits, stats);
    });
    if (valid) ctx->slots[ticket].busy = false;
    return rc;
}

static int search_now(swg_ctx *ctx, swg_db *db, bool allow_autotune, int32_t *scores_out, swg_hit *topk_out, size_t k,
                      size_t *n_hits, swg_stats *stats)
{
    if (k > 0 && !topk_out) return swg_set_ctx_error(ctx, SWG_ERR_ARG, "swg_search: k > 0 but topk_out NULL");
    int ticket = -1;
    const int rc = search_begin_ticket(ctx, db, scores_out != nullptr, k, allow_autotune, &ticket);
    if (rc != SWG_OK) return rc;
    return swg_search_end(ctx, ticket, scores_out, topk_out, n_hits, stats);
}

extern "C" int swg_search(swg_ctx *ctx, const swg_db *db, int32_t *scores_out, swg_hit *topk_out, size_t k,
                          size_t *n_hits, swg_stats *stats)
{
// ... 1818 lines not shown
```

seq-align-gpu_amd/csrc/swg_diag_host.cpp:

```cpp
#include "swg_host_internal.h"
#include "../../include/swg_host.h"

#include <algorithm>
#include <atomic>
#include <cmath>
#include <cstring>
#include <mutex>
#include <queue>

static std::mutex g_plan_cache_mutex;

static const double kCyclesPerInstr[5] = {0.0, 6.8, 4.55, 4.27, 4.35};
static const double kHotCycles = 13.0;

uint64_t swg_db_pair_count(const swg_db *db) { return (db->n_local + 1) / 2; }

uint64_t swg_db_pair_rows(const swg_db *db, uint64_t pair_begin, uint64_t pair_end, uint64_t *longest_rows)
{
    const uint64_t n = swg_db_pair_count(db);
    std::vector<uint64_t> &pre = const_cast<swg_db *>(db)->pair_rows_prefix;
    if (pre.size() != n + 1) {
        pre.assign(n + 1, 0);
        for (uint64_t p = 0; p < n; ++p) pre[p + 1] = pre[p] + 2ull + db->lens[2 * p];
    }
// ... 454 lines not shown
    uint64_t u = 0;
    for (size_t j = 0; j < len; ++j) u += cm.v[(uint8_t)seq[j] & 31];
    return u;
}

extern "C" int swg_debug_prune_bound(const int8_t *rows, const int8_t *idx, size_t lq, const int8_t *flat, const uint64_t *offsets, size_t n,
                                     uint8_t *colmax_out, uint64_t *u_out)
{
    if (!rows || lq == 0 || (n > 0 && (!flat || !offsets || !u_out))) return SWG_ERR_ARG;
    const SwgColMax cm = swg_prune_colmax(rows, idx, lq);
    if (colmax_out) memcpy(colmax_out, cm.v, 32);
    for (size_t i = 0; i < n; ++i) u_out[i] = swg_prune_bound(cm, flat + offsets[i], (size_t)(offsets[i + 1] - offsets[i]));
    return SWG_OK;
}

SwgPrunePlan swg_prune_plan(const SwgPruneAsk &a)
{
    SwgPrunePlan r;
    if (a.fixed) {
        if (a.mode == 0 || a.gap_open > 0 || a.gap_extend > 0 || a.bits != 16 || !a.use_diag || a.n_classes != 1 || !a.work_queue || a.both_forms ||
            a.gapless || a.batch || a.range_pairs == 0)
            return r;
        if (a.mode == 1 && !swg_prune_above_auto(a.range_pairs, a.groups)) return r;
        r.on = true;
        r.fixed = true;
        return r;
    }
    if (a.mode == 0 || a.k == 0 || a.k > SWG_TOPK_CAND_CAP / 2 || (a.want_scores && a.mode != 2) || a.gap_open > 0 || a.gap_extend > 0 ||
        a.bits != 16 || !a.use_diag || a.n_classes != 1 || !a.work_queue || a.both_forms || a.gapless || a.batch || a.range_pairs == 0 ||
        a.prune_head < 0)
        return r;
    const uint64_t need = ((uint64_t)a.k + 1) / 2, per_group = (uint64_t)a.prune_head * std::max<uint64_t>(1, a.groups);
    if (a.mode == 1 && (a.n_segments <= 1 || a.range_pairs < 4 * per_group)) return r;
    uint64_t head = 0;
    if (a.n_segments <= 1) {
        head = std::max(need, std::min(per_group, a.range_pairs / 4));
        if (head >= a.range_pairs) return r;
    }
    r.on = true;
    r.head_pairs = (uint32_t)head;
    return r;
}

extern "C" int swg_debug_prune_plan(const int64_t *in, int64_t *out)
{
    if (!in || !out || in[1] < 0 || in[12] < 0 || in[13] < 0 || in[15] < 0) return SWG_ERR_ARG;
    SwgPruneAsk a;
    a.mode = (int)in[0], a.k = (size_t)in[1], a.want_scores = in[2] != 0, a.gap_open = (int)in[3], a.gap_extend = (int)in[4];
    a.bits = (int)in[5], a.use_diag = in[6] != 0, a.n_classes = (int)in[7], a.work_queue = in[8] != 0, a.both_forms = in[9] != 0;
    a.gapless = in[10] != 0, a.batch = in[11] != 0, a.range_pairs = (uint64_t)in[12], a.groups = (uint64_t)in[13], a.prune_head = (long)in[14];
    a.n_segments = (size_t)in[15];
    const SwgPrunePlan r = swg_prune_plan(a);
    out[0] = r.on ? 1 : 0;
    out[1] = (int64_t)r.head_pairs;
    return SWG_OK;
}

extern "C" int swg_debug_prune_plan_above(const int64_t *in, int64_t *out)
{
    if (!in || !out || in[10] < 0 || in[11] < 0 || in[12] < 0) return SWG_ERR_ARG;
    SwgPruneAsk a;
    a.fixed = true;
    a.mode = (int)in[0], a.gap_open = (int)in[1], a.gap_extend = (int)in[2], a.bits = (int)in[3], a.use_diag = in[4] != 0, a.n_classes = (int)in[5];
    a.work_queue = in[6] != 0, a.both_forms = in[7] != 0, a.gapless = in[8] != 0, a.batch = in[9] != 0, a.range_pairs = (uint64_t)in[10];
    a.groups = (uint64_t)in[11], a.n_segments = (size_t)in[12], a.prune_head = (long)in[13];
    const SwgPrunePlan r = swg_prune_plan(a);
    out[0] = r.on ? 1 : 0;
    out[1] = (int64_t)r.head_pairs;
    return SWG_OK;
}

std::vector<SwgPruneStage> swg_prune_stages(const SwgPrunePlan &plan, const std::vector<std::pair<uint32_t, uint32_t>> &segments)
{
    std::vector<SwgPruneStage> stages;
    for (size_t i = 0; i < segments.size(); ++i) {
        const uint32_t b = segments[i].first, en = segments[i].second;
        const uint32_t mid = segments.size() == 1 && plan.head_pairs > 0 ? std::min(en, b + plan.head_pairs) : en;
        stages.push_back(SwgPruneStage{b, mid, (uint32_t)i, 0u});
        if (mid < en) stages.push_back(SwgPruneStage{mid, en, (uint32_t)i, 0u});
    }
    for (size_t si = 0; si < stages.size(); ++si) {
        if (si == 0 && !plan.fixed) continue;
        uint32_t q = plan.fixed ? 0u : SWG_STAGE_THRESHOLD;
        if (plan.prefix_cut) q |= SWG_STAGE_PREFIX_CUT;
        else {
            if (plan.refine && plan.fixed && si == 0 && stages.size() > 1) q |= SWG_STAGE_GATE;
            if (plan.refine) q |= SWG_STAGE_REFINE;
            if (plan.refine3) q |= SWG_STAGE_REFINE3;
            if (plan.refine4) q |= SWG_STAGE_REFINE4;
            q |= SWG_STAGE_LIST;
        }
        stages[si].queued = q;
    }
    return stages;
}

static int debug_prune_stages(const int64_t *in, int head, int64_t *out, size_t cap, size_t *n_out)
{
    if (!in || !n_out || (cap > 0 && !out) || in[0] < 0 || in[head - 1] < 0) return SWG_ERR_ARG;
    SwgPrunePlan plan;
    plan.on = true;
    plan.head_pairs = (uint32_t)in[0], plan.fixed = in[1] != 0, plan.refine = (int)in[2], plan.prefix_cut = in[3] != 0;
    plan.refine3 = head >= 6 ? (int)in[4] : 0;
    plan.refine4 = head == 7 ? (int)in[5] : 0;
    std::vector<std::pair<uint32_t, uint32_t>> segments;
    for (int64_t i = 0; i < in[head - 1]; ++i) segments.emplace_back((uint32_t)in[head + 2 * i], (uint32_t)in[head + 1 + 2 * i]);
    const std::vector<SwgPruneStage> stages = swg_prune_stages(plan, segments);
    for (size_t i = 0; i < stages.size() && i < cap; ++i)
        out[4 * i] = stages[i].begin, out[4 * i + 1] = stages[i].end, out[4 * i + 2] = stages[i].segment, out[4 * i + 3] = stages[i].queued;
    *n_out = stages.size();
    return SWG_OK;
}
extern "C" int swg_debug_prune_stages(const int64_t *in, int64_t *out, size_t cap, size_t *n_out) { return debug_prune_stages(in, 5, out, cap, n_out); }
extern "C" int swg_debug_prune_stages3(const int64_t *in, int64_t *out, size_t cap, size_t *n_out) { return debug_prune_stages(in, 6, out, cap, n_out); }
extern "C" int swg_debug_prune_stages4(const int64_t *in, int64_t *out, size_t cap, size_t *n_out) { return debug_prune_stages(in, 7, out, cap, n_out); }

void swg_kmer_cprof(const int8_t *rows, const int8_t *idx, size_t lq, int8_t *cprof)
{
    for (size_t i = 0; i < lq; ++i) {
        const int8_t *row = idx ? rows + 32 * ((uint8_t)idx[i] & 31) : rows + 32 * i;
        int8_t *out = cprof + SWG_KMER_CLASSES * i;
        for (uint32_t c = 0; c < SWG_KMER_CLASSES; ++c) out[c] = SWG_KMER_PAD_SCORE;
        for (uint32_t r = 1; r < 32; ++r) {
            const uint32_t c = swg_kmer_class(r);
            out[c] = std::max(out[c], row[r]);
        }
    }
}

static void kmer_row(const int8_t *cprof, size_t lq, int g, int e, size_t S, uint32_t c, const int *Mp, const int *Bp, const int *best_p, int *Mn,
                     int *Bn, int *best)
{
    const size_t W = (lq + S - 1) / S;
    int a = 0, up = 0;
    for (size_t s = 0; s < S; ++s) best[s] = best_p ? best_p[s] : 0;
    for (size_t s = 0, i = 0; i < lq; ++s) {
        int bs = best[s];
        for (const size_t end = std::min(lq, i + W); i < end; ++i) {
            const int sc = cprof[SWG_KMER_CLASSES * i + c];
            a = std::max(std::max(up - g, a - e), 0);
            const int b = Mp ? std::max(std::max(Mp[i] - g, Bp[i] - e), 0) : 0;
            const int diag = Mp && i ? Mp[i - 1] : 0;
            const int m = std::max(std::max(diag + sc, a), b);
            Mn[i] = m, Bn[i] = b, up = m;
            bs = std::max(bs, m);
        }
        best[s] = bs;
    }
}

static void kmer_extend(const int8_t *cprof, size_t lq, int g, int e, int k, size_t S, int depth, size_t prefix, const int *Mp, const int *Bp,
                        const int *best_p, std::vector<int> &work, uint16_t *table, uint32_t c_begin, uint32_t c_end)
{
    int *Mn = work.data() + (size_t)depth * (2 * lq + S), *Bn = Mn + lq, *best = Bn + lq;
    for (uint32_t c = c_begin; c < c_end; ++c) {
        kmer_row(cprof, lq, g, e, S, c, depth ? Mp : nullptr, Bp, best_p, Mn, Bn, best);
        const size_t at = prefix * SWG_KMER_CLASSES + c;
        if (depth + 1 == k)
            for (size_t s = 0; s < S; ++s) table[at * S + s] = (uint16_t)std::min(best[s], 65535);
        else kmer_extend(cprof, lq, g, e, k, S, depth + 1, at, Mn, Bn, best, work, table, 0, SWG_KMER_CLASSES);
    }
}

void swg_kmer_table_seg(const int8_t *cprof, size_t lq, int g, int e, int k, size_t S, uint16_t *table)
{
    g = std::min(g, 65536), e = std::min(e, 65536);
#pragma omp parallel for schedule(dynamic, 1)
    for (int c = 0; c < (int)SWG_KMER_CLASSES; ++c) {
        std::vector<int> work((size_t)k * (2 * lq + S));
        kmer_extend(cprof, lq, g, e, k, S, 0, 0, nullptr, nullptr, nullptr, work, table, (uint32_t)c, (uint32_t)c + 1u);
    }
}

template <class Entries>
static uint64_t kmer_bound_walk(Entries entries, int k, size_t S, const SwgColMax &cm, const int8_t *seq, size_t len)
{
    const size_t n_blocks = (2 + len + 3) / 4, n_rows = 4 * n_blocks;
    auto res = [&](size_t row) -> uint32_t { return row < 2 || row >= 2 + len ? 0u : (uint8_t)seq[row - 2] & 31u; };
    const size_t rows5 = k == 5 ? 20 * (n_blocks / 5) : 0;
    std::vector<uint64_t> H(S, 0);
    for (size_t r = 0; r < n_rows;) {
        const size_t rows = r < rows5 ? 5 : 4;
        size_t ix = 0;
        uint64_t sum = 0, run = 0;
        for (size_t j = 0; j < rows; ++j) ix = ix * SWG_KMER_CLASSES + swg_kmer_class(res(r + j)), sum += cm.v[res(r + j)];
        if (k == 5 && rows == 4) ix *= SWG_KMER_CLASSES;
        const uint16_t *t = entries(ix);
        for (size_t s = 0; s < S; ++s) {
            run = std::max(run, H[s]);
            H[s] = run + std::min<uint64_t>(t[s], sum);
        }
        r += rows;
    }
    return *std::max_element(H.begin(), H.end());
}

uint64_t swg_kmer_bound_seg(const uint16_t *table, int k, size_t S, const SwgColMax &cm, const int8_t *seq, size_t len)
{
// ... 120 lines not shown
            auto gain = [&](const SwgKmerCandidate &c) { return c.gain * (double)a.pair_rows / a.fill_rate; };
            const SwgKmerCandidate *cur = &SWG_KMER_CANDIDATES[0];
            for (const SwgKmerCandidate &c : SWG_KMER_CANDIDATES) {
                if (forced_S && c.S != 1) continue;
                if (c.gain > cur->gain && cost(c) - cost(*cur) <= 0.5 * (gain(c) - gain(*cur))) cur = &c;
            }
            k = cur->k, S_out = cur->S;
            if (forced_S && k > 1) {
                if (k == 5 && !swg_kmer_table_admitted(5, forced_S)) k = 4;
                S_out = (int)forced_S;
            }
        }
    }
    if (segments) *segments = k > 1 ? S_out : (k ? 1 : 0);
    return k;
}

static bool debug_kmer_ask(const int64_t *in, int64_t *out, int n_in, SwgKmerAsk *a)
{
    if (!in || !out) return false;
    for (int i = 2; i < std::min(n_in, 7); ++i)
        if (in[i] < 0) return false;
    if (n_in > 7 && !swg_prune_refine_value_ok((long)in[7])) return false;
    a->forced = (long)in[0], a->pruned = in[1] != 0, a->lq = (size_t)in[2], a->pair_rows = (uint64_t)in[3];
    a->table_rate = in[4] ? (double)in[4] : SWG_KMER_TABLE_RATE;
    a->fill_rate = in[5] ? (double)in[5] : swg_kmer_fill_rate(a->lq);
    a->forced_segments = n_in > 6 ? (long)in[6] : 1;
    a->forced_refine = n_in > 7 ? (long)in[7] : 0;
    return true;
}
extern "C" int swg_debug_prune_kmer_choice(const int64_t *in, int64_t *out)
{
    SwgKmerAsk a;
    if (!debug_kmer_ask(in, out, 6, &a)) return SWG_ERR_ARG;
    out[0] = swg_prune_kmer_choice(a);
    return SWG_OK;
}
extern "C" int swg_debug_prune_kmer_choice_seg(const int64_t *in, int64_t *out)
{
    SwgKmerAsk a;
    if (!debug_kmer_ask(in, out, 7, &a)) return SWG_ERR_ARG;
    int S = 0;
    out[0] = swg_prune_kmer_choice(a, &S);
    out[1] = S;
    out[2] = (int64_t)(swg_kmer_entries((int)out[0]) * (uint64_t)S * sizeof(uint16_t));
    out[3] = out[0] <= 1 || swg_kmer_table_admitted((int)out[0], S) ? 1 : 0;
    return SWG_OK;
}

struct SwgRefineCandidate {
    int S2;
    double gain, bound_row;
};
static const SwgRefineCandidate SWG_REFINE_CANDIDATES[] = {{0, 0.0, 0.0}, {64, 0.0234, 2.1e-12}, {128, 0.0428, 2.1e-12}};
int swg_prune_refine_choice(const SwgKmerAsk &a, int k, int S)
{
    if (!a.pruned || k < 1) return 0;
    if (a.forced_refine == 64 || a.forced_refine == 128) return (int)a.forced_refine;
    if (a.forced_refine != 0 || a.forced != 0 || a.forced_segments != 0 || k != 4 || S <= 1) return 0;
    if (a.table_rate <= 0 || a.fill_rate <= 0 || a.lq == 0) return 0;
    auto cost = [&](const SwgRefineCandidate &c) {
        return c.S2 == 0 ? 0.0 : (double)swg_kmer_entries(4) * 4 * (double)a.lq / a.table_rate + c.bound_row * (double)a.pair_rows;
    };
    auto gain = [&](const SwgRefineCandidate &c) { return c.gain * (double)a.pair_rows / a.fill_rate; };
    const SwgRefineCandidate *cur = &SWG_REFINE_CANDIDATES[0];
    for (const SwgRefineCandidate &c : SWG_REFINE_CANDIDATES)
        if (c.gain > cur->gain && cost(c) - cost(*cur) <= 0.5 * (gain(c) - gain(*cur))) cur = &c;
    return cur->S2;
}

extern "C" int swg_debug_prune_refine_choice(const int64_t *in, int64_t *out)
{
    SwgKmerAsk a;
    if (!debug_kmer_ask(in, out, 8, &a)) return SWG_ERR_ARG;
    int S = 0;
    out[0] = swg_prune_kmer_choice(a, &S);
    out[1] = S;
    out[2] = swg_prune_refine_choice(a, (int)out[0], S);
    return SWG_OK;
}

#define SWG_REFINE3_GAIN 0.0151
#define SWG_REFINE3_BOUND_ROW 1.74e-12
int swg_prune_refine3_choice(const SwgKmerAsk &a, int k, int S, int S2)
{
    if (!a.pruned || k < 1) return 0;
    if (a.forced_refine3 == 256) return 256;
    if (a.forced_refine3 != 0 || a.forced != 0 || a.forced_segments != 0 || a.forced_refine != 0) return 0;
    if (k != 4 || S <= 1 || S2 != 128 || a.table_bits != 8) return 0;
    if (a.table_rate <= 0 || a.fill_rate <= 0 || a.lq == 0) return 0;
    const double cost = (double)swg_kmer_entries(4) * 4 * (double)a.lq / a.table_rate + SWG_REFINE3_BOUND_ROW * (double)a.pair_rows;
    const double gain = SWG_REFINE3_GAIN * (double)a.pair_rows / a.fill_rate;
    return cost <= 0.5 * gain ? 256 : 0;
}

extern "C" int swg_debug_prune_refine3_choice(const int64_t *in, int64_t *out)
{
    SwgKmerAsk a;
    if (!debug_kmer_ask(in, out, 8, &a)) return SWG_ERR_ARG;
    if (!swg_prune_refine3_value_ok((long)in[8]) || (in[9] != 0 && in[9] != 8 && in[9] != 16)) return SWG_ERR_ARG;
    a.forced_refine3 = (long)in[8];
    a.table_bits = in[9] == 16 ? 16 : 8;
    int S = 0;
    out[0] = swg_prune_kmer_choice(a, &S);
    out[1] = S;
    out[2] = swg_prune_refine_choice(a, (int)out[0], S);
    out[3] = swg_prune_refine3_choice(a, (int)out[0], S, (int)out[2]);
    return SWG_OK;
}

#define SWG_REFINE4_GAIN 0.0374
#define SWG_REFINE4_BOUND_ROW 1.31e-12
int swg_prune_refine4_choice(const SwgKmerAsk &a, int k, int S, int S2, int S3)
{
    if (!a.pruned || k < 1 || !swg_kmer_refine4_admitted(a.table_bits5)) return 0;
    if (a.forced_refine4 == SWG_REFINE4_FORCED) return (int)SWG_KMER_REFINE4_SEGMENTS;
    if (a.forced_refine4 != 0 || a.forced != 0 || a.forced_segments != 0 || a.forced_refine != 0 || a.forced_refine3 != 0) return 0;
    if (k != 4 || S <= 1 || S2 != 128 || S3 != 256 || a.table_bits != 8) return 0;
    if (a.table_rate <= 0 || a.fill_rate <= 0 || a.lq == 0) return 0;
    const double cost = swg_kmer_table_cells(5) * (double)a.lq / a.table_rate + SWG_REFINE4_BOUND_ROW * (double)a.pair_rows;
    const double gain = SWG_REFINE4_GAIN * (double)a.pair_rows / a.fill_rate;
    return cost <= 0.5 * gain ? (int)SWG_KMER_REFINE4_SEGMENTS : 0;
}

extern "C" int swg_debug_prune_refine4_choice(const int64_t *in, int64_t *out)
{
    SwgKmerAsk a;
    if (!debug_kmer_ask(in, out, 8, &a)) return SWG_ERR_ARG;
    if (!swg_prune_refine3_value_ok((long)in[8]) || (in[9] != 0 && in[9] != 8 && in[9] != 16)) return SWG_ERR_ARG;
    if (!swg_prune_refine4_value_ok((long)in[10]) || (in[11] != 0 && in[11] != 8 && in[11] != 16)) return SWG_ERR_ARG;
    a.forced_refine3 = (long)in[8], a.forced_refine4 = (long)in[10];
    a.table_bits = in[9] == 16 ? 16 : 8, a.table_bits5 = in[11] == 16 ? 16 : 8;
    int S = 0;
    out[0] = swg_prune_kmer_choice(a, &S);
    out[1] = S;
    out[2] = swg_prune_refine_choice(a, (int)out[0], S);
    out[3] = swg_prune_refine3_choice(a, (int)out[0], S, (int)out[2]);
    out[4] = swg_prune_refine4_choice(a, (int)out[0], S, (int)out[2], (int)out[3]);
    return SWG_OK;
}

uint32_t swg_split_rows(size_t lq, uint64_t qbound)
{
    if (qbound == 0) return 0u;
    return (uint32_t)std::min<uint64_t>(((uint64_t)SWG_F16_CEILING * lq + qbound - 1) / qbound, 1u << 30);
}

void swg_db_split_at(swg_db *db, uint32_t rows)
{
    if (db->split_rows == rows) return;
    const size_t n = db->lens.size();
    const size_t first_short = (size_t)(std::partition_point(db->lens.begin(), db->lens.end(), [rows](uint32_t l) { return l >= rows; }) -
                                        db->lens.begin());
    db->split_rows = rows;
    db->split_pair = (uint32_t)((first_short + 1) / 2);
    uint64_t sum = 0;
    for (size_t i = std::min(n, (size_t)db->split_pair * 2); i < n; ++i) sum += db->lens[i];
    db->split_residues = sum;
}

extern "C" int swg_debug_split(swg_db *db, size_t lq, uint64_t qbound, uint64_t *out)
{
    if (!db || !out || lq == 0 || qbound == 0) return SWG_ERR_ARG;
    const uint32_t rows = swg_split_rows(lq, qbound);
    swg_db_split_at(db, rows);
    out[0] = rows;
    out[1] = db->split_pair;
    out[2] = db->split_residues;
    return SWG_OK;
}

double swg_systolic_estimate_ms(const swg_db *db, size_t lq, int n_cu, int *best_K, bool f16)
{
    *best_K = 0;
    if (db->n_bins == 0 || db->bin_nblk.size() != db->n_bins) return 1e300;
    uint64_t blocks = 0;
// ... 157 lines not shown
```

seq-align-gpu_amd/csrc/swg_host_internal.h:

```cpp
#pragma once
#include "../../include/swg.h"
#include "swg_internal.h"

#include <algorithm>
#include <functional>
#include <map>
#include <memory>
#include <new>
#include <string>
#include <utility>
#include <vector>

template <class T> struct SwgNoInit {
    using value_type = T;
    SwgNoInit() = default;
    template <class U> SwgNoInit(const SwgNoInit<U> &) {}
    T *allocate(size_t n) { return static_cast<T *>(::operator new(n * sizeof(T))); }
    void deallocate(T *p, size_t) { ::operator delete(p); }
    template <class U> void construct(U *p) noexcept { ::new ((void *)p) U; }
    template <class U, class A0, class... A> void construct(U *p, A0 &&a0, A &&...a)
    {
        ::new ((void *)p) U(std::forward<A0>(a0), std::forward<A>(a)...);
    }
    template <class U> bool operator==(const SwgNoInit<U> &) const { return true; }
// ... 99 lines not shown
    bool masked = false;
    swg_mask_info mask_info = {};
    swg_db *root = nullptr;
    std::vector<uint32_t> root_slot;
    size_t refs = 1;
    bool handle_live = true;
    std::vector<uint32_t> slot_of;
    int device = -1;
    uint32_t *d_codes = nullptr;
    uint64_t *d_code_off = nullptr;
    uint32_t *d_lens = nullptr;
    uint32_t *d_order = nullptr;
    uint32_t *d_packed = nullptr;
    uint64_t *d_bin_off = nullptr;
    uint32_t *d_bin_nblk = nullptr;
    uint64_t upload_bytes = 0;
    struct Bufs {
        int32_t *d_scores = nullptr;
        uint32_t *d_list = nullptr;
        uint32_t *d_counters = nullptr;
        uint64_t *d_keys = nullptr;
        uint32_t *d_hist = nullptr;
        uint32_t *d_pair_bound = nullptr;
        size_t pair_bound_cap = 0;
        uint64_t *d_above = nullptr;
        size_t above_cap = 0;
    } bufs[4];
    int32_t *d_scores = nullptr;
    uint32_t *d_list = nullptr;
    uint32_t *d_counters = nullptr;
    uint64_t *d_keys = nullptr;
    uint32_t *d_hist = nullptr;
    uint32_t *d_pair_bound = nullptr;
    std::vector<uint32_t> prune_stages;
};

#define SWG_F16_GAP_MAX 2048
#define SWG_F16_CEILING 4096
#define SWG_I16_CEILING 32767
#define SWG_WIDE_CEILING 65535
inline bool swg_f16_gaps_ok(int go, int ge) { return -go <= SWG_F16_GAP_MAX && -ge <= SWG_F16_GAP_MAX; }

#define SWG_LDS_PER_CU ((size_t)160 * 1024)
inline int swg_workgroups_per_cu(int wave_budget, int W, size_t lds)
{
    return std::max(1, std::min<int>(wave_budget / W, (int)(SWG_LDS_PER_CU / lds)));
}

struct SwgScoreBound {
    uint64_t qbound = 0, bound = 0;
    int smax = 0;
};
SwgScoreBound swg_score_bound(const int8_t *rows, const int8_t *idx, size_t lq, uint64_t longest);
extern "C" int swg_debug_score_bound(const int8_t *rows, const int8_t *idx, size_t lq, uint64_t longest, uint64_t *out);

SwgColMax swg_prune_colmax(const int8_t *rows, const int8_t *idx, size_t lq);
uint64_t swg_prune_bound(const SwgColMax &cm, const int8_t *seq, size_t len);
struct SwgPruneAsk {
    int mode = 1;
    size_t k = 0;
    bool want_scores = false;
    int gap_open = 0, gap_extend = 0;
    int bits = 16;
    bool use_diag = true;
    int n_classes = 1;
    bool work_queue = true;
    bool both_forms = false;
    bool gapless = false;
    bool batch = false;
    uint64_t range_pairs = 0, groups = 0;
    long prune_head = 4;
    size_t n_segments = 1;
    bool fixed = false;
};
struct SwgPrunePlan {
    bool on = false;
    uint32_t head_pairs = 0;
    int kmer = 0;
    int segments = 0;
    int refine = 0;
    int refine3 = 0;
    int refine4 = 0;
    bool prefix_cut = false;
    bool fixed = false;
    uint32_t fixed_T = 0;
};
#define SWG_PRUNE_STAGE_RECS 256u
struct SwgPruneLayout {
    uint32_t *bounds, *ids, *lists, *tiles, *recs;
    size_t words;
};
inline SwgPruneLayout swg_prune_layout(uint32_t *base, size_t n_pairs)
{
    const size_t tiles = 3 * n_pairs, recs = tiles + n_pairs / SWG_PRUNE_TILE + 2;
    auto at = [base](size_t word) { return base ? base + word : nullptr; };
    return SwgPruneLayout{base, at(n_pairs), at(2 * n_pairs), at(tiles), at(recs), recs + 2 * SWG_PRUNE_STAGE_RECS};
}
SwgPrunePlan swg_prune_plan(const SwgPruneAsk &a);
enum : uint32_t {
    SWG_STAGE_THRESHOLD = 1u, SWG_STAGE_PREFIX_CUT = 2u, SWG_STAGE_GATE = 4u, SWG_STAGE_REFINE = 8u, SWG_STAGE_LIST = 16u, SWG_STAGE_REFINE3 = 32u,
    SWG_STAGE_REFINE4 = 64u
};
struct SwgPruneStage {
    uint32_t begin, end;
    uint32_t segment;
    uint32_t queued;
};
std::vector<SwgPruneStage> swg_prune_stages(const SwgPrunePlan &plan, const std::vector<std::pair<uint32_t, uint32_t>> &segments);
extern "C" int swg_debug_prune_stages(const int64_t *in, int64_t *out, size_t cap, size_t *n_out);
extern "C" int swg_debug_prune_stages3(const int64_t *in, int64_t *out, size_t cap, size_t *n_out);
extern "C" int swg_debug_prune_stages4(const int64_t *in, int64_t *out, size_t cap, size_t *n_out);
#define SWG_PRUNE_ABOVE_AUTO_PAIRS 16u
inline bool swg_prune_above_auto(uint64_t range_pairs, uint64_t groups) { return range_pairs >= SWG_PRUNE_ABOVE_AUTO_PAIRS * std::max<uint64_t>(1, groups); }
inline int swg_above_multi_route(long option, bool admitted, bool single_pruned)
{
    if (option == 2 || !admitted) return 2;
    if (option == 1) return 1;
    return single_pruned ? 2 : 1;
}
extern "C" int swg_debug_above_multi_route(long option, int admitted, int single_pruned);
extern "C" int swg_debug_prune_bound(const int8_t *rows, const int8_t *idx, size_t lq, const int8_t *flat, const uint64_t *offsets, size_t n,
                                     uint8_t *colmax_out, uint64_t *u_out);
extern "C" int swg_debug_prune_plan(const int64_t *in, int64_t *out);
extern "C" int swg_debug_prune_plan_above(const int64_t *in, int64_t *out);
void swg_kmer_cprof(const int8_t *rows, const int8_t *idx, size_t lq, int8_t *cprof);
void swg_kmer_table_seg(const int8_t *cprof, size_t lq, int g, int e, int k, size_t S, uint16_t *table);
uint64_t swg_kmer_bound_seg(const uint16_t *table, int k, size_t S, const SwgColMax &cm, const int8_t *seq, size_t len);
#define SWG_KMER_TABLE_RATE 4.6e12
#define SWG_KMER_FILL_PASS_RATE 9.4e9
inline double swg_kmer_table_cells(int k)
{
    return k == 5 ? (double)swg_kmer_entries(4) * (4 + SWG_KMER_CLASSES) : (double)swg_kmer_entries(k) * k;
}
inline double swg_kmer_fill_rate(size_t lq) { return SWG_KMER_FILL_PASS_RATE / (double)std::max<size_t>(1, (lq + 511) / 512); }
struct SwgKmerAsk {
    long forced = 0;
    long forced_segments = 0;
    long forced_refine = 0;
    long forced_refine3 = 0;
    long forced_refine4 = 0;
    int table_bits5 = 8;
    int table_bits = 8;
    bool pruned = false;
    size_t lq = 0;
    uint64_t pair_rows = 0;
    double table_rate = SWG_KMER_TABLE_RATE, fill_rate = 0;
};
inline bool swg_kmer_table_admitted(int k, long S)
{
    return S >= 1 && S <= (long)SWG_KMER_MAX_SEGMENTS && swg_kmer_entries(k) * (uint64_t)S * sizeof(uint16_t) <= SWG_KMER_TABLE_BUDGET;
}
int swg_prune_kmer_choice(const SwgKmerAsk &a, int *segments = nullptr);
extern "C" int swg_debug_prune_kmer(const int8_t *rows, const int8_t *idx, size_t lq, int gap_open, int gap_extend, int k, const int8_t *flat,
                                    const uint64_t *offsets, size_t n, uint16_t *table_out, uint64_t *u_out);
extern "C" int swg_debug_prune_kmer_seg(const int8_t *rows, const int8_t *idx, size_t lq, int gap_open, int gap_extend, int k, int S,
                                        const int8_t *flat, const uint64_t *offsets, size_t n, uint16_t *table_out, uint64_t *u_out);
extern "C" int swg_debug_prune_kmer_choice(const int64_t *in, int64_t *out);
extern "C" int swg_debug_prune_kmer_choice_seg(const int64_t *in, int64_t *out);
int swg_prune_refine_choice(const SwgKmerAsk &a, int k, int S);
inline bool swg_prune_refine_value_ok(long v) { return v == 0 || v == 1 || v == 64 || v == 128; }
extern "C" int swg_debug_prune_refine_choice(const int64_t *in, int64_t *out);
extern "C" int swg_debug_prune_kmer_refine(const int8_t *rows, const int8_t *idx, size_t lq, int gap_open, int gap_extend, int S2, const int8_t *flat,
                                           const uint64_t *offsets, size_t n, uint16_t *table_out, uint64_t *u_out);
int swg_prune_refine3_choice(const SwgKmerAsk &a, int k, int S, int S2);
inline bool swg_prune_refine3_value_ok(long v) { return v == 0 || v == 1 || v == 256; }
extern "C" int swg_debug_prune_refine3_choice(const int64_t *in, int64_t *out);
extern "C" int swg_debug_prune_kmer_refine3(const int8_t *rows, const int8_t *idx, size_t lq, int gap_open, int gap_extend, int S3, const int8_t *flat,
                                            const uint64_t *offsets, size_t n, uint16_t *table_out, uint64_t *u_out);
extern "C" int swg_debug_prune_table_bits(const int8_t *rows, const int8_t *idx, size_t lq, int k);
#define SWG_REFINE4_FORCED 5256
int swg_prune_refine4_choice(const SwgKmerAsk &a, int k, int S, int S2, int S3);
inline bool swg_prune_refine4_value_ok(long v) { return v == 0 || v == 1 || v == SWG_REFINE4_FORCED; }
extern "C" int swg_debug_prune_refine4_choice(const int64_t *in, int64_t *out);
extern "C" int swg_debug_prune_kmer_refine4(const int8_t *rows, const int8_t *idx, size_t lq, int gap_open, int gap_extend, int S4, const int8_t *flat,
                                            const uint64_t *offsets, size_t n, uint64_t *u_out);
#define SWG_PRUNE_WORD_T 18u
#define SWG_PRUNE_WORD_CUT 20u
#define SWG_ABOVE_WORD_COUNT 24u
#define SWG_PRUNE_WORD_GATE 25u
#define SWG_ABOVE_KEYS_FLOOR SWG_TOPK_CAND_CAP

struct SwgSystolicPlan {
    int bits = 0, variant = 0, K = 0, W = 0, npass = 0, workgroups = 0;
    SwgKernelInfo info = {};
    int f16 = 0;
};

struct SwgSearchPlan {
    int bits = 0;
    bool fast_ok = false;
    int go = 0, ge = 0;
    int go32 = 0, ge32 = 0;
    bool gapless = false;
    bool gapless_cells = false;
    uint64_t score_bound = ~0ull, qbound = 0;
    uint64_t epoch = 0;
    bool use_f16 = false;
    bool wide = false;
    uint32_t split_at = 0, split_rows = 0;
    uint64_t split_residues = 0;
    bool rerun_wide = false;
    int32_t ceiling = 0;
    int32_t level_ceiling = 0;
    bool may_saturate = false;
    bool int32_level = false;
    bool q32_ok = false;
    bool bin32 = false;
    bool some_f16() const { return use_f16 || split_at != 0u; }
    bool use_diag = false, use_diag32 = false, use_q32 = false, exact32 = false;
    SwgDiagWork wk, wk32;
    SwgSystolicPlan main_pl, re_pl;
    int npass32 = 0;
    SwgPrunePlan prune;
};

struct SwgBatchPlan {
    bool one_launch = false;
    int go = 0, ge = 0;
    int form = 0;
    bool qq = false;
    SwgDiagWork wk;
    int qq_per_cu = 1;
    uint64_t bound_max = 0;
    size_t lq_max = 0;
    bool dev_topk = false;
    size_t n_slots = 0;
    size_t chunk_queries = 0, first_chunk = 0;
    size_t grid_rows(size_t Qb) const { return qq ? (Qb + 1) / 2 : Qb; }
    size_t score_rows(size_t Qb) const { return qq ? 2 * grid_rows(Qb) : Qb; }
    size_t score_rows_cap = 0, grid_rows_cap = 0;
    size_t order_entries = 0;
    uint32_t class_queue_dwords = 0;
    size_t rank_word_base = 0, queue_dwords = 0;
    size_t prof_row_bytes[2] = {0, 0};
};

struct SwgKmerTable {
    uint8_t *d = nullptr;
    size_t cap = 0;
    uint64_t epoch = 0;
    int k = 0, segments = 0;
    int bits = 0;
    bool holds(uint64_t e, int k_, int S, int bits_) const { return d && epoch == e && k == k_ && segments == S && bits == bits_; }
};
struct SwgPruneChoice {
    int kmer = 0, segments = 0, refine = 0, refine3 = 0, refine4 = 0;
};

#define SWG_MAX_INFLIGHT 4
struct SwgSlot {
    hipEvent_t ev[8] = {nullptr, nullptr, nullptr, nullptr, nullptr, nullptr, nullptr, nullptr};
    hipEvent_t ev_done = nullptr;
    SwgSearchPlan plan;
    bool side = false;
    bool busy = false;
    swg_db *db = nullptr;
    swg_db::Bufs bufs;
    size_t k = 0, first_chunk = 0;
    bool want_scores = false, dev_topk = false, need_scores = false, two_ends = false;
    int fill_launches = 0;
    bool pruned = false;
    int32_t above_min = 0;
    size_t above_cap = 0;
    int fill_f16_launches = 0;
    swg_stats st;
    uint64_t *h_cand = nullptr;
    uint32_t *h_counters = nullptr;
    int32_t *h_scores = nullptr;
    size_t h_scores_cap = 0;
};

struct SwgBatch16Cache {
    swg_db *db = nullptr;
    size_t slots_cap = 0, pairs_cap = 0, stage_cap = 0;
    uint64_t blocks_cap = 0;
    uint8_t *h_stage = nullptr, *d_stage = nullptr;
    uint8_t *h_meta = nullptr;
    uint64_t *d_pair_src = nullptr;
    uint32_t *d_pair_len = nullptr;
};

struct swg_ctx {
    int device = 0;
    hipStream_t stream = nullptr;
    hipStream_t stream2 = nullptr;
    hipStream_t stream3 = nullptr;
    int n_cu = 0;
    unsigned long n_begun = 0;
    std::string err;
    bool have_scoring = false;
    int8_t sub[32][32];
    int gap_open = 0, gap_extend = 0;
    std::vector<int8_t> query;
    int8_t *h_query_stage[4] = {nullptr, nullptr, nullptr, nullptr};
    size_t h_query_stage_cap[4] = {0, 0, 0, 0};
    hipEvent_t ev_query_stage[4] = {nullptr, nullptr, nullptr, nullptr};
    int query_stage_next = 0;
    std::vector<int8_t> pssm;
    bool query_pssm = false;
    bool gapless = false;
    int32_t above_min = 0;
    size_t query_len() const { return query_pssm ? pssm.size() / 32 : query.size(); }
    long opt_force_bits = 0, opt_cols = 0, opt_max_waves = 0, opt_workgroups = 0, opt_engine = 0, opt_group = 0, opt_long_split = 0, opt_autotune = 1, opt_dynamic = 1, opt_prio_share = 150, opt_long_helps = 0, opt_wide = 1, opt_side_readout = 1, opt_f16 = 1, opt_qq = 1, opt_last_pass = 1, opt_f16_pair = 0;
    long opt_batch_geometry = 0;
    long opt_wave_budget = 0, opt_q32_waves = 0;
    long opt_bounds_groups = 0;
    uint32_t bounds_last[4] = {0, 0, 0, 0};
    long opt_batch = 8, opt_batch_blocks = 0;
    long opt_prune = 1, opt_prune_head = 4;
    bool in_batch = false;
    long opt_above_batch = 0;
    swg_prune_info prune_last = {};
    SwgPruneChoice prune_choice;
    SwgColMax prune_colmax;
    uint64_t prune_colmax_epoch = 0;
    long opt_prune_kmer = 0;
    long opt_prune_segments = 0;
    long opt_prune_refine = 0;
    long opt_prune_refine3 = 0;
    long opt_prune_refine4 = 0;
    long opt_prune_table_bits = 0;
    long opt_prune_cut = 0;
    int8_t *d_kmer_cprof = nullptr;
    size_t d_kmer_cprof_cap = 0;
    SwgKmerTable kmer_first[2], kmer_second, kmer_third, kmer_fourth;
    uint64_t kmer_builds = 0, kmer_refine_builds = 0, kmer_refine3_builds = 0, kmer_refine4_builds = 0;
    bool kmer_fourth_refused = false;
    uint32_t opt_seg_blocks = SWG_DYN_SEG_BLOCKS;
    int8_t *d_sub = nullptr;
    int8_t *d_query = nullptr;
    size_t d_query_cap = 0;
    int8_t *d_pssm = nullptr;
    size_t d_pssm_cap = 0;
    uint8_t *d_profile[8] = {nullptr, nullptr, nullptr, nullptr, nullptr, nullptr, nullptr, nullptr};
    size_t d_profile_cap[8] = {0, 0, 0, 0, 0, 0, 0, 0};
    uint64_t profile_tag[8] = {0, 0, 0, 0, 0, 0, 0, 0};
    uint64_t epoch = 1;
    uint32_t *d_scratch = nullptr;
    size_t d_scratch_cap = 0;
    SwgBatch16Cache b16;
    long opt_calib_seqs = 8192, opt_calib_len = 384, opt_calib_seed = 1;
    struct {
        swg_db *db = nullptr;
        double freq[32] = {};
        long seqs = 0, len = 0, seed = 0;
    } calib;
    std::vector<int32_t> calib_iters;
    long opt_pssm_msa_mb = 1024;
    SwgSlot slots[SWG_MAX_INFLIGHT];
    SwgSlot *cur = nullptr;
    int next_slot = 0;
};

#define SWG_TAKE_HOST_ROUTE 1
int swg_set_global_error(int code, const char *fmt, ...) __attribute__((format(printf, 2, 3)));
int swg_set_ctx_error(swg_ctx *ctx, int code, const char *fmt, ...)
    __attribute__((format(printf, 3, 4)));
void swg_db_release_device(swg_db *db);
void swg_db_release_search_state(swg_db *db);
inline const uint8_t *swg_db_codes(const swg_db *db) { return (db->root ? db->root : db)->codes.data(); }
int swg_view_select(const swg_db *parent, const uint32_t *indices, size_t n, std::vector<uint32_t> *slots,
                    std::vector<uint8_t> *marks = nullptr);
swg_db *swg_view_host(swg_db *parent, const std::vector<uint32_t> &slots);
size_t swg_db_views_alive(const swg_db *db);
extern "C" int swg_debug_view_ranks(const swg_db *db, const uint32_t *indices, size_t n, uint32_t *out, size_t *n_out);
struct SwgListJobs {
    std::vector<uint32_t> slots;
    std::vector<uint64_t> row_pairs;
    std::vector<uint32_t> entry_job;
    std::vector<uint64_t> row_residues;
    std::vector<uint32_t> row_longest;
    std::vector<uint64_t> pair_blocks;
    uint64_t entry0 = 0;
};
int swg_list_jobs(const swg_db *db, const uint32_t *cand, const uint64_t *c_off, size_t q0, size_t nq, SwgListJobs *J);
void swg_lists_deal(const SwgListJobs &J, uint64_t per_wg, uint64_t resident, bool equal_shares, std::vector<uint2> *out);
extern "C" int swg_debug_list_deal(const swg_db *db, const uint32_t *cand, const uint64_t *c_off, size_t n_queries, uint64_t per_wg,
                                   uint64_t resident, uint32_t *out, size_t cap, size_t *n_wgs);
extern "C" int swg_debug_list_jobs(const swg_db *db, const uint32_t *cand, const uint64_t *c_off, size_t n_queries, uint32_t *slots_out,
                                   size_t cap, size_t *n_slots, uint64_t *row_pairs_out);
extern "C" void swg_debug_fail_alloc(int site);
extern "C" int swg_debug_plan(const swg_db *db, size_t lq, int n_cu, int32_t *out);
extern "C" int swg_debug_plan_gapless(const swg_db *db, size_t lq, int n_cu, int32_t *out);
extern "C" int swg_debug_plan_f16(const swg_db *db, size_t lq, int n_cu, long f16_pair, int32_t *out);
extern "C" int swg_debug_plan_forced(const swg_db *db, size_t lq, int n_cu, long cols, long group, long waves, int form,
                                     long f16_pair, int last_pass, int32_t *out);
extern "C" int swg_debug_plan_streams(const swg_db *db, const int8_t *rows, const int8_t *idx, size_t lq, int n_cu, long cols, long group,
                                      long waves, long workgroups, int32_t *out);
extern "C" int swg_debug_plan_systolic(const swg_db *db, const int8_t *rows, const int8_t *idx, size_t lq, int gap_open, int gap_extend, int n_cu,
                                       long force_bits, long cols, long max_waves, long workgroups, long f16, int32_t *out);
extern "C" int swg_debug_systolic_variants(int bits, int32_t *out, size_t cap);
extern "C" int swg_debug_plan_batch(const swg_db *db, size_t lq_max, size_t n_queries, int n_cu, int form, int qq_on, long cols, long group,
                                    long batch_geometry, int32_t *out);
extern "C" int swg_debug_plan_lists(const uint32_t *pair_lens, size_t n_pairs, size_t lq_max, int n_cu, int form, long cols, long group,
                                    long batch_geometry, int32_t *out);
#define SWG_LAUNCH_LOG_CAP 4096
#define SWG_LAUNCH_LOG_FIELDS 10
extern "C" void swg_debug_launch_log(int on);
extern "C" size_t swg_debug_launch_log_read(int32_t *out, size_t cap);
#define SWG_SYSTOLIC_MARGIN 0.85
double swg_systolic_estimate_ms(const swg_db *db, size_t lq, int n_cu, int *best_K, bool f16 = false);
double swg_diag_short_pair_factor(const swg_db *db, const SwgDiagPlan &pl, int form);
extern "C" int swg_debug_engine(const swg_db *db, size_t lq, int n_cu, int form, int32_t *out);
// ... 79 lines not shown
```

seq-align-gpu_amd/csrc/swg_internal.h:

```cpp
#pragma once
#include <hip/hip_runtime.h>
#include <stdint.h>

#define SWG_BIN 128
#define SWG_ROWS_PER_BLK 4
#define SWG_BIN_COLUMN(s) ((((s)&1u) * 64u) + ((s) >> 1))

struct SwgFillParams {
    const uint32_t *residues;
    const uint64_t *bin_off;
    const uint32_t *bin_nblk;
    uint32_t n_bins;
    const uint8_t *profile;
    int32_t *scores;
    uint32_t *queue;
    const uint32_t *list;
    const uint32_t *list_count;
    uint32_t n_items;
    uint32_t npass;
    int32_t go, ge;
    uint32_t *scratch;
    uint64_t scratch_wg_dwords;
};

// ... 139 lines not shown
hipError_t swg_launch_diag_lists(int variant, int form, int W, int workgroups, const SwgDiagDynParams &p, hipStream_t stream);
hipError_t swg_launch_build_profiles_multi(const int8_t *d_sub, const int8_t *d_queries, const uint32_t *d_q_off,
                                           uint32_t n_queries, uint32_t ncols, int k_real, int k_padded,
                                           uint8_t *d_profiles, hipStream_t stream, int swizzle_lanes = 0, int f16 = 0,
                                           const int8_t *d_pssms = nullptr);

#ifndef SWG_LDS_SWIZZLE
#define SWG_LDS_SWIZZLE 1
#endif

hipError_t swg_launch_build_profile(const int8_t *d_sub, const int8_t *d_query,
                                    uint32_t lq, uint32_t ncols, int elem_size, int chunk_cols, int k_real,
                                    int k_padded, uint8_t *d_profile, hipStream_t stream, int swizzle_lanes = 0,
                                    int f16 = 0,
                                    uint32_t qcol0 = 0,
                                    const int8_t *d_pssm = nullptr);
int swg_diag_padded_cols(int K, bool fma = false);
size_t swg_diag_slice_bytes(int K, int G, bool fma = false);

hipError_t swg_launch_build_tokens(const uint32_t *d_codes, const uint64_t *d_code_off, const uint32_t *d_lens,
                                   const uint32_t *d_pair_off, uint32_t n_pairs, uint64_t total_blocks, uint4 *d_tok,
                                   hipStream_t stream);
hipError_t swg_launch_build_tokens16(const uint8_t *d_stage, const uint64_t *d_pair_src, const uint32_t *d_pair_len,
                                     const uint32_t *d_pair_off, uint32_t n_pairs, uint64_t total_blocks, uint4 *d_tok,
                                     uint32_t *d_bad, hipStream_t stream);
hipError_t swg_launch_build_bins(const uint32_t *d_codes, const uint64_t *d_code_off, const uint32_t *d_lens,
                                 const uint64_t *d_bin_off, const uint32_t *d_bin_nblk, uint32_t n_bins,
                                 uint32_t *d_packed, hipStream_t stream);

hipError_t swg_launch_gather_view(const uint32_t *d_slots, uint32_t n_slots, uint32_t parent_slots, const uint64_t *p_code_off,
                                  const uint32_t *p_lens, const uint32_t *p_order, uint64_t *d_code_off, uint32_t *d_lens,
                                  uint32_t *d_order, hipStream_t stream);

hipError_t swg_launch_zero2(void *a, size_t a_bytes, void *b, size_t b_bytes, hipStream_t stream);
hipError_t swg_launch_collect_flagged_pairs(const int32_t *d_scores, uint32_t first_pair, uint32_t n_pairs, int32_t ceiling,
                                            uint32_t *d_list, uint32_t *d_count, uint32_t *d_seqs, const uint32_t *d_lens,
                                            uint32_t *d_rows16, hipStream_t stream);
hipError_t swg_launch_collect_saturated(const int32_t *d_scores, uint32_t n_slots, int32_t ceiling,
                                        uint32_t *d_list, uint32_t *d_count, const uint32_t *d_lens, uint32_t *d_rows16,
                                        hipStream_t stream);

#define SWG_TOPK_CAND_CAP 8192u
hipError_t swg_launch_topk(const int32_t *d_scores, const uint32_t *d_order, uint32_t n_slots, uint32_t k,
                           uint32_t *d_hist, uint32_t *d_thr, uint64_t *d_cand, uint32_t cap, uint32_t *d_count,
                           hipStream_t stream);
hipError_t swg_launch_above_compact(const int32_t *d_scores, const uint32_t *d_order, uint32_t n_slots, int32_t min_score, uint64_t *d_keys, uint32_t cap,
                                    uint32_t *d_count, hipStream_t stream);
hipError_t swg_launch_above_rows_count(const int32_t *d_scores, uint64_t row_stride, const uint32_t *d_order, uint32_t n_slots, uint32_t n_rows,
                                       const int32_t *d_thr, uint32_t *d_counts, hipStream_t stream);
hipError_t swg_launch_above_rows_scatter(const int32_t *d_scores, uint64_t row_stride, const uint32_t *d_order, uint32_t n_slots, uint32_t n_rows,
                                         const int32_t *d_thr, const uint32_t *d_counts, const uint64_t *d_offsets, uint32_t *d_cursors,
                                         uint64_t *d_keys, uint64_t keys_cap, hipStream_t stream);
struct SwgColMax {
    uint8_t v[32];
};
hipError_t swg_launch_pair_bound(const uint4 *d_tok, const uint32_t *d_pair_off, uint32_t n_pairs, const SwgColMax &cm,
                                 uint32_t *d_bound, uint32_t *d_ids, hipStream_t stream);
#define SWG_KMER_CLASSES 22u
#define SWG_KMER_STD_MASK 0x2DF7BFAu
#define SWG_KMER_PAD_SCORE (-128)
static inline __host__ __device__ uint32_t swg_kmer_class(uint32_t r)
{
    r &= 31u;
    if (r == 0u) return 0u;
    if (!((SWG_KMER_STD_MASK >> r) & 1u)) return SWG_KMER_CLASSES - 1u;
    uint32_t c = 0u;
    for (uint32_t i = 1u; i <= r; ++i) c += (SWG_KMER_STD_MASK >> i) & 1u;
    return c;
}
static inline uint64_t swg_kmer_entries(int k) { return k == 5 ? 5153632ull : k == 4 ? 234256ull : 0ull; }
#define SWG_KMER_MAX_SEGMENTS 32u
#define SWG_KMER_REFINE_SEGMENTS 256u
#define SWG_KMER_TABLE_BUDGET (96ull << 20)
static inline int swg_kmer_table_bits(const SwgColMax &cm, int k)
{
    uint32_t m = 0u;
    for (int r = 0; r < 32; ++r) m = cm.v[r] > m ? cm.v[r] : m;
    return (uint32_t)k * m <= 255u ? 8 : 16;
}
hipError_t swg_launch_kmer_table(const int8_t *d_sub, const int8_t *d_query, const int8_t *d_pssm, uint32_t lq, uint32_t g, uint32_t e,
                                 int k, uint32_t S, int8_t *d_cprof, void *d_table, int bits, hipStream_t stream);
hipError_t swg_launch_pair_bound_kmer(const uint4 *d_tok, const uint32_t *d_pair_off, uint32_t n_pairs, int k, const SwgColMax &cm,
                                      const void *d_table, int bits, uint32_t *d_bound, uint32_t *d_ids, hipStream_t stream);
hipError_t swg_launch_pair_bound_kmer_seg(const uint4 *d_tok, const uint32_t *d_pair_off, uint32_t n_pairs, int k, uint32_t S, const SwgColMax &cm,
                                          const void *d_table, int bits, uint32_t *d_bound, uint32_t *d_ids, hipStream_t stream);
hipError_t swg_launch_prune_threshold(const int32_t *d_scores, const uint32_t *d_order, uint32_t n_slots, uint32_t k, uint32_t *d_hist,
                                      uint32_t *d_thr, hipStream_t stream);
hipError_t swg_launch_prune_cut(const uint32_t *d_bound, const uint32_t *d_pair_off, uint32_t begin, uint32_t end, const uint32_t *d_thr,
                                uint32_t *d_out, hipStream_t stream);
hipError_t swg_launch_pair_bound_refine(const uint4 *d_tok, const uint32_t *d_pair_off, uint32_t begin, uint32_t end, uint32_t S2, const SwgColMax &cm,
                                        const void *d_table, int bits, const uint32_t *d_thr, uint32_t *d_bound, hipStream_t stream, int k = 4);
#define SWG_KMER_REFINE4_SEGMENTS 256u
#define SWG_KMER_REFINE4_BUDGET (2ull << 30)
static inline bool swg_kmer_refine4_admitted(int bits) { return bits == 8 && swg_kmer_entries(5) * SWG_KMER_REFINE4_SEGMENTS <= SWG_KMER_REFINE4_BUDGET; }
#define SWG_PRUNE_TILE 1024u
hipError_t swg_launch_prune_refine_gate(const uint32_t *d_bound, uint32_t begin, uint32_t end, const uint32_t *d_thr, uint32_t *d_gate, hipStream_t stream);
hipError_t swg_launch_prune_list(const uint32_t *d_bound, const uint32_t *d_pair_off, uint32_t begin, uint32_t end, const uint32_t *d_thr,
                                 uint32_t *d_tiles, uint32_t *d_list, uint32_t *d_out, uint32_t *d_rec, hipStream_t stream);
#define SWG_TOPK_MULTI_CAP 1024u
hipError_t swg_launch_topk_multi(const int32_t *d_scores, uint64_t score_stride, const uint32_t *d_order, uint32_t n_slots,
                                 uint32_t n_queries, uint32_t k, uint32_t *d_hist, uint32_t *d_meta, uint64_t *d_cand, uint32_t cap,
                                 hipStream_t stream);

hipError_t swg_launch_db_composition(const uint32_t *d_codes, const uint64_t *d_code_off, const uint32_t *d_lens, uint32_t n_slots,
                                     unsigned long long *d_counts, hipStream_t stream);
#define SWG_CALIB_BINS 4096u
struct SwgCalibFit {
    double lambda, mu;
    int32_t n_iter, status;
    uint32_t n, reserved;
};
hipError_t swg_launch_calib_fit(const int32_t *d_scores, uint64_t row_stride, const uint32_t *d_order, uint32_t n_slots, uint32_t n_rows,
                                SwgCalibFit *d_out, hipStream_t stream);
```

seq-align-gpu_amd/csrc/swg_kernels.hip:

```cpp
#include "swg_internal.h"
#include <type_traits>

#ifdef SWG_PART
#define SWG_HAS_PART(n) (SWG_PART == (n))
#else
#define SWG_HAS_PART(n) 1
#endif
#ifdef SWG_PROBE_VARIANT
#define SWG_APPLY(X, ...) X(__VA_ARGS__)
#define SWG_DIAG_VARIANTS(X) SWG_APPLY(X, SWG_PROBE_VARIANT)
#else
#define SWG_DIAG_VARIANTS(X)                                                                                          \
    X(24, 16) X(12, 16) X(8, 16) X(16, 16) X(32, 12) X(6, 16) X(10, 16) X(20, 16) X(28, 12) X(4, 16) X(14, 16) X(18, 16) \
    X(22, 16) X(2, 16) X(23, 16) X(21, 16) X(19, 16) X(17, 16) X(15, 16) X(13, 16) X(11, 16) X(9, 16) X(7, 16) X(31, 12)  \
    X(29, 12) X(27, 12) X(25, 12) X(30, 12) X(26, 12) X(5, 16) X(3, 16)
#endif

typedef short s16x2 __attribute__((ext_vector_type(2)));
typedef unsigned short u16x2 __attribute__((ext_vector_type(2)));

#define DEVINL __device__ __forceinline__

DEVINL uint32_t pk_add_i16_sat(uint32_t a, uint32_t b)
{
// ... 2614 lines not shown
            ux += block4(lut[(k.x >> 3) & 31u], lut[(k.y >> 3) & 31u], lut[(k.z >> 3) & 31u], lut[(k.w >> 3) & 31u]);
            uy += block4(lut[(k.x >> 11) & 31u], lut[(k.y >> 11) & 31u], lut[(k.z >> 11) & 31u], lut[(k.w >> 11) & 31u]);
        }
    }
#pragma unroll
    for (int d = 8; d >= 1; d >>= 1) {
        ux += (uint32_t)__shfl_xor((int)ux, d, 16);
        uy += (uint32_t)__shfl_xor((int)uy, d, 16);
    }
    if (p < n_pairs && l == 0u) {
        bound[p] = ux > uy ? ux : uy;
        ids[p] = p;
    }
}

hipError_t swg_launch_pair_bound_kmer(const uint4 *d_tok, const uint32_t *d_pair_off, uint32_t n_pairs, int k, const SwgColMax &cm,
                                      const void *d_table, int bits, uint32_t *d_bound, uint32_t *d_ids, hipStream_t stream)
{
    if ((k != 4 && k != 5) || (bits != 8 && bits != 16)) return hipErrorInvalidValue;
    if (n_pairs == 0) return hipSuccess;
    const dim3 grid((n_pairs + 15u) / 16u);
    const uint8_t *t8 = static_cast<const uint8_t *>(d_table);
    const uint16_t *t16 = static_cast<const uint16_t *>(d_table);
    if (k == 5 && bits == 8)
        hipLaunchKernelGGL((swg_pair_bound_kmer_kernel<5, uint8_t>), grid, dim3(256), 0, stream, d_tok, d_pair_off, n_pairs, cm, t8, d_bound, d_ids);
    else if (k == 5)
        hipLaunchKernelGGL((swg_pair_bound_kmer_kernel<5, uint16_t>), grid, dim3(256), 0, stream, d_tok, d_pair_off, n_pairs, cm, t16, d_bound, d_ids);
    else if (bits == 8)
        hipLaunchKernelGGL((swg_pair_bound_kmer_kernel<4, uint8_t>), grid, dim3(256), 0, stream, d_tok, d_pair_off, n_pairs, cm, t8, d_bound, d_ids);
    else
        hipLaunchKernelGGL((swg_pair_bound_kmer_kernel<4, uint16_t>), grid, dim3(256), 0, stream, d_tok, d_pair_off, n_pairs, cm, t16, d_bound, d_ids);
    return hipGetLastError();
}

template <int WD>
__device__ __forceinline__ uint32_t swg_seg_prefix_max(uint32_t h, uint32_t m1, uint32_t m2, uint32_t m4)
{
    uint32_t t = (uint32_t)__builtin_amdgcn_update_dpp(0, (int)h, 0x111, 0xf, 0xf, true);
    if (WD == 8) t &= m1;
    h = t > h ? t : h;
    t = (uint32_t)__builtin_amdgcn_update_dpp(0, (int)h, 0x112, 0xf, 0xf, true);
    if (WD == 8) t &= m2;
    h = t > h ? t : h;
    t = (uint32_t)__builtin_amdgcn_update_dpp(0, (int)h, 0x114, 0xf, 0xf, true);
    if (WD == 8) t &= m4;
    h = t > h ? t : h;
    if (WD >= 16) {
        t = (uint32_t)__builtin_amdgcn_update_dpp(0, (int)h, 0x118, 0xf, 0xf, true);
        h = t > h ? t : h;
    }
    if (WD == 32) {
        t = (uint32_t)__builtin_amdgcn_update_dpp(0, (int)h, 0x142, 0xa, 0xf, false);
        h = t > h ? t : h;
    }
    return h;
}

template <int WD, int NB, int U, class E>
__device__ __forceinline__ void swg_seg_chunk(const uint32_t (&ux)[NB], const uint32_t (&uy)[NB], const uint32_t (&uc)[NB], uint32_t cnt,
                                              const E *tl, uint32_t S, bool has, uint32_t m1, uint32_t m2, uint32_t m4, uint32_t &hx,
                                              uint32_t &hy)
{
    for (uint32_t j0 = 0u; j0 < cnt; j0 += (uint32_t)U) {
        uint32_t tx[U * NB], ty[U * NB], cs[U * NB];
#pragma unroll
        for (int u = 0; u < U; ++u)
#pragma unroll
            for (int b = 0; b < NB; ++b) {
                const int src = (int)j0 + u;
                const uint32_t ix = (uint32_t)__shfl((int)ux[b], src, WD), iy = (uint32_t)__shfl((int)uy[b], src, WD);
                cs[u * NB + b] = (uint32_t)__shfl((int)uc[b], src, WD);
                tx[u * NB + b] = has ? (uint32_t)tl[ix * S] : 0u;
                ty[u * NB + b] = has ? (uint32_t)tl[iy * S] : 0u;
            }
#pragma unroll
        for (int i = 0; i < U * NB; ++i) {
            const uint32_t cx = cs[i] & 0xFFFFu, cy = cs[i] >> 16;
            hx = swg_seg_prefix_max<WD>(hx, m1, m2, m4) + (tx[i] < cx ? tx[i] : cx);
            hy = swg_seg_prefix_max<WD>(hy, m1, m2, m4) + (ty[i] < cy ? ty[i] : cy);
        }
    }
}

template <int K, int WD, class E>
__global__ __launch_bounds__(256) void swg_pair_bound_kmer_seg_kernel(const uint4 *tok, const uint32_t *pair_off, uint32_t n_pairs, SwgColMax cm,
                                                                      const E *table, uint32_t S, uint32_t *bound, uint32_t *ids)
{
    __shared__ uint32_t lut[32];
    if (threadIdx.x < 32u) lut[threadIdx.x] = swg_kmer_class(threadIdx.x) | (uint32_t)cm.v[threadIdx.x] << 8;
    __syncthreads();
    const uint32_t p = blockIdx.x * (256u / WD) + threadIdx.x / WD, l = threadIdx.x & (WD - 1u);
    const uint32_t C = SWG_KMER_CLASSES;
    const bool has = l < S;
    const E *tl = table + (has ? l : 0u);
    const uint32_t m1 = (l & 7u) >= 1u ? 0xFFFFFFFFu : 0u, m2 = (l & 7u) >= 2u ? 0xFFFFFFFFu : 0u, m4 = (l & 7u) >= 4u ? 0xFFFFFFFFu : 0u;
    uint32_t hx = 0u, hy = 0u;
    if (p < n_pairs) {
        const uint32_t b0 = pair_off[p], e = pair_off[p + 1u];
        uint32_t tail = b0;
        if (K == 5) {
            const uint32_t groups = (e - b0) / 5u;
            tail = b0 + 5u * groups;
            for (uint32_t g0 = 0u; g0 < groups; g0 += WD) {
                uint32_t ux[4] = {0u, 0u, 0u, 0u}, uy[4] = {0u, 0u, 0u, 0u}, uc[4] = {0u, 0u, 0u, 0u};
                if (g0 + l < groups) {
                    uint32_t x[20], y[20];
#pragma unroll
                    for (int u = 0; u < 5; ++u) {
                        const uint4 k = tok[b0 + 5u * (g0 + l) + (uint32_t)u];
                        x[4 * u] = lut[(k.x >> 3) & 31u], x[4 * u + 1] = lut[(k.y >> 3) & 31u], x[4 * u + 2] = lut[(k.z >> 3) & 31u], x[4 * u + 3] = lut[(k.w >> 3) & 31u];
                        y[4 * u] = lut[(k.x >> 11) & 31u], y[4 * u + 1] = lut[(k.y >> 11) & 31u], y[4 * u + 2] = lut[(k.z >> 11) & 31u], y[4 * u + 3] = lut[(k.w >> 11) & 31u];
                    }
#pragma unroll
                    for (int u = 0; u < 4; ++u) {
                        uint32_t ix = 0u, iy = 0u, sx = 0u, sy = 0u;
#pragma unroll
                        for (int j = 0; j < 5; ++j) {
                            ix = ix * C + (x[5 * u + j] & 255u), sx += x[5 * u + j] >> 8;
                            iy = iy * C + (y[5 * u + j] & 255u), sy += y[5 * u + j] >> 8;
                        }
                        ux[u] = ix, uy[u] = iy, uc[u] = sx | sy << 16;
                    }
                }
                swg_seg_chunk<WD, 4, 1>(ux, uy, uc, groups - g0 < WD ? groups - g0 : WD, tl, S, has, m1, m2, m4, hx, hy);
            }
        }
        for (uint32_t t0 = tail; t0 < e; t0 += WD) {
            uint32_t ux[1] = {0u}, uy[1] = {0u}, uc[1] = {0u};
            if (t0 + l < e) {
                const uint4 k = tok[t0 + l];
                const uint32_t xa = lut[(k.x >> 3) & 31u], xb = lut[(k.y >> 3) & 31u], xc = lut[(k.z >> 3) & 31u], xd = lut[(k.w >> 3) & 31u];
                const uint32_t ya = lut[(k.x >> 11) & 31u], yb = lut[(k.y >> 11) & 31u], yc = lut[(k.z >> 11) & 31u], yd = lut[(k.w >> 11) & 31u];
                const uint32_t ix = (((xa & 255u) * C + (xb & 255u)) * C + (xc & 255u)) * C + (xd & 255u);
                const uint32_t iy = (((ya & 255u) * C + (yb & 255u)) * C + (yc & 255u)) * C + (yd & 255u);
                ux[0] = K == 5 ? ix * C : ix, uy[0] = K == 5 ? iy * C : iy;
                uc[0] = ((xa >> 8) + (xb >> 8) + (xc >> 8) + (xd >> 8)) | ((ya >> 8) + (yb >> 8) + (yc >> 8) + (yd >> 8)) << 16;
            }
            swg_seg_chunk<WD, 1, 4>(ux, uy, uc, e - t0 < WD ? e - t0 : WD, tl, S, has, m1, m2, m4, hx, hy);
        }
    }
    const uint32_t h = hx > hy ? hx : hy, u = swg_seg_prefix_max<WD>(h, m1, m2, m4);
    if (p < n_pairs && l == WD - 1u) {
        bound[p] = u;
        ids[p] = p;
    }
}

template <int K, class E>
static void swg_launch_pair_bound_kmer_seg_k(const uint4 *d_tok, const uint32_t *d_pair_off, uint32_t n_pairs, const SwgColMax &cm,
                                             const E *d_table, uint32_t S, uint32_t *d_bound, uint32_t *d_ids, hipStream_t stream)
{
    if (S <= 8u)
        hipLaunchKernelGGL((swg_pair_bound_kmer_seg_kernel<K, 8, E>), dim3((n_pairs + 31u) / 32u), dim3(256), 0, stream, d_tok, d_pair_off, n_pairs, cm, d_table, S, d_bound, d_ids);
    else if (S <= 16u)
        hipLaunchKernelGGL((swg_pair_bound_kmer_seg_kernel<K, 16, E>), dim3((n_pairs + 15u) / 16u), dim3(256), 0, stream, d_tok, d_pair_off, n_pairs, cm, d_table, S, d_bound, d_ids);
    else
        hipLaunchKernelGGL((swg_pair_bound_kmer_seg_kernel<K, 32, E>), dim3((n_pairs + 7u) / 8u), dim3(256), 0, stream, d_tok, d_pair_off, n_pairs, cm, d_table, S, d_bound, d_ids);
}

hipError_t swg_launch_pair_bound_kmer_seg(const uint4 *d_tok, const uint32_t *d_pair_off, uint32_t n_pairs, int k, uint32_t S, const SwgColMax &cm,
                                          const void *d_table, int bits, uint32_t *d_bound, uint32_t *d_ids, hipStream_t stream)
{
    if ((k != 4 && k != 5) || S == 0u || S > SWG_KMER_MAX_SEGMENTS || (bits != 8 && bits != 16)) return hipErrorInvalidValue;
    if (n_pairs == 0) return hipSuccess;
    const uint8_t *t8 = static_cast<const uint8_t *>(d_table);
    const uint16_t *t16 = static_cast<const uint16_t *>(d_table);
    if (k == 5 && bits == 8)
        swg_launch_pair_bound_kmer_seg_k<5>(d_tok, d_pair_off, n_pairs, cm, t8, S, d_bound, d_ids, stream);
    else if (k == 5)
        swg_launch_pair_bound_kmer_seg_k<5>(d_tok, d_pair_off, n_pairs, cm, t16, S, d_bound, d_ids, stream);
    else if (bits == 8)
        swg_launch_pair_bound_kmer_seg_k<4>(d_tok, d_pair_off, n_pairs, cm, t8, S, d_bound, d_ids, stream);
    else
        swg_launch_pair_bound_kmer_seg_k<4>(d_tok, d_pair_off, n_pairs, cm, t16, S, d_bound, d_ids, stream);
    return hipGetLastError();
}

hipError_t swg_launch_prune_threshold(const int32_t *d_scores, const uint32_t *d_order, uint32_t n_slots, uint32_t k, uint32_t *d_hist,
                                      uint32_t *d_thr, hipStream_t stream)
{
    hipError_t e = hipMemsetAsync(d_hist, 0, SWG_TOPK_BINS * sizeof(uint32_t), stream);
    if (e != hipSuccess) return e;
    const int blocks = (int)((n_slots + 255) / 256 < 512 ? (n_slots + 255) / 256 : 512);
    hipLaunchKernelGGL(swg_topk_hist_kernel, dim3(blocks > 0 ? blocks : 1), dim3(256), 0, stream, d_scores, d_order, n_slots, d_hist,
                       (uint64_t)0);
    hipLaunchKernelGGL(swg_topk_threshold_kernel, dim3(1), dim3(SWG_TOPK_THR_THREADS), 0, stream, d_hist, k, 0xFFFFFFFFu, d_thr);
    return hipGetLastError();
}

#define SWG_PRUNE_CUT_THREADS 256
__global__ __launch_bounds__(SWG_PRUNE_CUT_THREADS) void swg_prune_cut_kernel(const uint32_t *bound, uint32_t begin, uint32_t end, const uint32_t *thr,
                                                                              uint32_t *out)
{
    const uint32_t T = thr[0];
    uint32_t m = 0u;
    for (uint64_t p = (uint64_t)begin + blockIdx.x * SWG_PRUNE_CUT_THREADS + threadIdx.x; p < end; p += (uint64_t)gridDim.x * SWG_PRUNE_CUT_THREADS)
        if (bound[p] >= T) m = (uint32_t)p + 1u - begin;
#pragma unroll
    for (int d = 32; d >= 1; d >>= 1) {
        const uint32_t o = (uint32_t)__shfl_xor((int)m, d, 64);
        m = o > m ? o : m;
    }
    if ((threadIdx.x & 63u) == 0u && m > 0u) atomicMax(out, m);
}

__global__ void swg_prune_tally_kernel(const uint32_t *pair_off, uint32_t begin, uint32_t end, uint32_t *out)
{
    if (blockIdx.x != 0u || threadIdx.x != 0u) return;
    const uint32_t cut = begin + out[0];
    out[1] += end - cut;
    *reinterpret_cast<unsigned long long *>(out + 2) += (unsigned long long)(pair_off[end] - pair_off[cut]);
}

hipError_t swg_launch_prune_cut(const uint32_t *d_bound, const uint32_t *d_pair_off, uint32_t begin, uint32_t end, const uint32_t *d_thr,
                                uint32_t *d_out, hipStream_t stream)
{
    if (end < begin) return hipErrorInvalidValue;
    hipError_t e = hipMemsetAsync(d_out, 0, sizeof(uint32_t), stream);
    if (e != hipSuccess) return e;
    const uint32_t per_wg = SWG_PRUNE_CUT_THREADS * 8u;
    const uint32_t want = (end - begin + per_wg - 1u) / per_wg;
    const uint32_t wgs = want < 1u ? 1u : want > 1024u ? 1024u : want;
    hipLaunchKernelGGL(swg_prune_cut_kernel, dim3(wgs), dim3(SWG_PRUNE_CUT_THREADS), 0, stream, d_bound, begin, end, d_thr, d_out);
    hipLaunchKernelGGL(swg_prune_tally_kernel, dim3(1), dim3(64), 0, stream, d_pair_off, begin, end, d_out);
    return hipGetLastError();
}

template <int PL>
__device__ __forceinline__ void swg_refine_step(uint32_t (&h)[PL], const uint32_t (&t)[PL], uint32_t m0)
{
    uint32_t pm[PL];
    pm[0] = h[0];
#pragma unroll
    for (int j = 1; j < PL; ++j) pm[j] = h[j] > pm[j - 1] ? h[j] : pm[j - 1];
    uint32_t ex = (uint32_t)__builtin_amdgcn_update_dpp(0, (int)pm[PL - 1], 0x138, 0xf, 0xf, true) & m0;
    ex = swg_seg_prefix_max<32>(ex, 0u, 0u, 0u);
#pragma unroll
    for (int j = 0; j < PL; ++j) h[j] = (ex > pm[j] ? ex : pm[j]) + t[j];
}

template <int PL>
__device__ __forceinline__ void swg_refine_entries(const uint16_t *at, uint32_t c, uint32_t (&t)[PL])
{
    uint32_t w[4] = {0u, 0u, 0u, 0u};
    if (PL == 8) {
        const uint4 v = *reinterpret_cast<const uint4 *>(at);
        w[0] = v.x, w[1] = v.y, w[2] = v.z, w[3] = v.w;
    } else if (PL == 4) {
        const uint2 v = *reinterpret_cast<const uint2 *>(at);
        w[0] = v.x, w[1] = v.y;
    } else {
        w[0] = *reinterpret_cast<const uint32_t *>(at);
    }
#pragma unroll
    for (int j = 0; j < PL; ++j) {
        const uint32_t e = j & 1 ? w[j / 2] >> 16 : w[j / 2] & 0xFFFFu;
        t[j] = e < c ? e : c;
// ... 636 lines not shown
```

Measured before the change: 48820.

## Gate segmented k-mer bound on a cheap column-max bound after threshold

Moves the segmented k-mer first-level bound kernel to run after the top-k threshold is known on non-head stages. It first computes a cheap per-pair column-max bound and skips the expensive segmented table walk for pairs already below the threshold. Pairs in the head range are marked not-bounded, so their bound is never computed. The aim is to cut bound-computation cost on pruned searches, at the cost of reordering the stage schedule, adding a reduction per pair, and a cost-model gate that reuses the refine3 heuristic.

```diff
diff --git a/seq-align-gpu_amd/__init__.py b/seq-align-gpu_amd/__init__.py
--- a/seq-align-gpu_amd/__init__.py
+++ b/seq-align-gpu_amd/__init__.py
@@ -293,6 +293,9 @@
 _sig("swg_debug_prune_tables4", C.c_int, [_vp, _vp])
 _sig("swg_debug_prune_refine4_read", C.c_int, [_vp, _vp, C.c_size_t, _vp])
 _sig("swg_debug_prune_refine4_choice", C.c_int, [_vp, _vp])
+_sig("swg_debug_prune_gate_choice", C.c_int, [_vp, _vp])
+_sig("swg_debug_prune_gate", C.c_int, [_vp, _vp])
+_sig("swg_debug_prune_stages5", C.c_int, [_vp, _vp, C.c_size_t, _vp])
 _sig("swg_debug_prune_stages4", C.c_int, [_vp, _vp, C.c_size_t, C.POINTER(C.c_size_t)])
 _sig("swg_debug_list_deal", C.c_int, [_vp, _vp, _vp, C.c_size_t, C.c_uint64, C.c_uint64, _vp, C.c_size_t, C.POINTER(C.c_size_t)])
 _sig("swg_debug_calib_iters", C.c_int, [_vp, _vp, C.c_size_t, C.POINTER(C.c_size_t)])
@@ -701,6 +704,13 @@
     return tuple(int(v) for v in out)
 
 
+def debug_prune_gate_choice(forced=0, segments=0, gate=0, pruned=1, lq=3000, pair_rows=1900000000, table_rate=0, fill_rate=0):
+    a = np.array([forced, pruned, lq, pair_rows, table_rate, fill_rate, segments, 0, gate], dtype=np.int64)
+    out = np.zeros(3, dtype=np.int64)
+    _check(lib.swg_debug_prune_gate_choice(a.ctypes.data_as(_vp), out.ctypes.data_as(_vp)))
+    return int(out[0]), int(out[1]), bool(out[2])
+
+
 def debug_prune_refine_choice(forced=0, segments=0, refine=0, pruned=1, lq=3000, pair_rows=1900000000, table_rate=0, fill_rate=0):
     a = np.array([forced, pruned, lq, pair_rows, table_rate, fill_rate, segments, refine], dtype=np.int64)
     out = np.zeros(3, dtype=np.int64)
@@ -755,14 +765,16 @@
 
 
 PRUNE_STAGE_QUEUED = ("threshold", "prefix_cut", "gate", "refine", "list")
-_PRUNE_STAGE_BITS = ((0, "threshold"), (1, "prefix_cut"), (2, "gate"), (3, "refine"), (5, "refine3"), (6, "refine4"), (4, "list"))
-
-
-def debug_prune_stages(segments, head_pairs=0, fixed=False, refine=0, prefix_cut=False, refine3=0, refine4=0):
-    a = np.array([head_pairs, fixed, refine, prefix_cut, refine3, refine4, len(segments)] + [int(v) for sg in segments for v in sg], dtype=np.int64)
+_PRUNE_STAGE_BITS = ((0, "threshold"), (7, "bound"), (1, "prefix_cut"), (2, "gate"), (3, "refine"), (5, "refine3"), (6, "refine4"), (4, "list"))
+
+
+def debug_prune_stages(segments, head_pairs=0, fixed=False, refine=0, prefix_cut=False, refine3=0, refine4=0, gate=False):
+    head = [head_pairs, fixed, refine, prefix_cut, refine3, refine4] + ([1] if gate else [])
+    a = np.array(head + [len(segments)] + [int(v) for sg in segments for v in sg], dtype=np.int64)
     out = np.zeros((2 * len(segments) + 1, 4), dtype=np.int64)
     n = C.c_size_t(0)
-    _check(lib.swg_debug_prune_stages4(a.ctypes.data_as(_vp), out.ctypes.data_as(_vp), out.shape[0], C.byref(n)))
+    hook = lib.swg_debug_prune_stages5 if gate else lib.swg_debug_prune_stages4
+    _check(hook(a.ctypes.data_as(_vp), out.ctypes.data_as(_vp), out.shape[0], C.byref(n)))
     return [(int(b), int(e), int(sg), tuple(name for i, name in _PRUNE_STAGE_BITS if int(qd) >> i & 1))
             for b, e, sg, qd in out[:n.value]]
 
@@ -1500,6 +1512,11 @@
         _check(lib.swg_debug_prune_tables4(self.handle, out.ctypes.data_as(_vp)), self.handle)
         return {"refine4": int(out[0]), "refine4_builds": int(out[1]), "bits": int(out[2]), "refused": bool(out[3])}
 
+    def debug_prune_gate(self):
+        out = np.zeros(1, dtype=np.int64)
+        _check(lib.swg_debug_prune_gate(self.handle, out.ctypes.data_as(_vp)), self.handle)
+        return bool(out[0])
+
     def debug_prune_refine4_read(self, blocks):
         b = np.ascontiguousarray(blocks, dtype=np.uint32)
         out = np.zeros((max(b.size, 1), KMER_REFINE4_SEGMENTS), dtype=np.uint16)
diff --git a/seq-align-gpu_amd/csrc/swg_api.cpp b/seq-align-gpu_amd/csrc/swg_api.cpp
--- a/seq-align-gpu_amd/csrc/swg_api.cpp
+++ b/seq-align-gpu_amd/csrc/swg_api.cpp
@@ -331,6 +331,10 @@
         if (!swg_prune_refine4_value_ok(value))
             return swg_set_ctx_error(ctx, SWG_ERR_ARG, "prune_refine4 must be 0 (auto), 1 (off) or 5256 (the fourth-level bound's table: k = 5 in 256 segments)");
         ctx->opt_prune_refine4 = value;
+    } else if (!strcmp(key, "prune_gate")) {
+        if (!swg_prune_gate_value_ok(value))
+            return swg_set_ctx_error(ctx, SWG_ERR_ARG, "prune_gate must be 0 (auto), 1 (off) or 2 (wherever the first-level bound is a segmented k-mer bound)");
+        ctx->opt_prune_gate = value;
     } else if (!strcmp(key, "prune_table_bits")) {
         if (value != 0 && value != 16)
             return swg_set_ctx_error(ctx, SWG_ERR_ARG, "prune_table_bits must be 0 (auto: bytes where they hold every entry) or 16");
@@ -1129,19 +1133,33 @@
     uint32_t *thr = db->d_counters + SWG_PRUNE_WORD_T, *cut_word = db->d_counters + SWG_PRUNE_WORD_CUT, *gate = db->d_counters + SWG_PRUNE_WORD_GATE;
     const uint32_t n_pairs = (uint32_t)swg_db_pair_count(db);
     const SwgPruneLayout L = swg_prune_layout(db->d_pair_bound, n_pairs);
-    if (pr.kmer > 1 && pr.segments > 1)
-        HIP_TRY(ctx, swg_launch_pair_bound_kmer_seg(T.d_tok, T.d_pair_off, n_pairs, pr.kmer, (uint32_t)pr.segments, ctx->prune_colmax, ctx->kmer_first[pr.kmer - 4].d,
+    if (pr.fixed) HIP_TRY(ctx, hipMemsetD32Async(reinterpret_cast<hipDeviceptr_t>(thr), (int)pr.fixed_T, 1, qs));
+    const std::vector<SwgPruneStage> stages = swg_prune_stages(pr, F->segs);
+    auto first_level = [&](uint32_t b, uint32_t en, const uint32_t *gated_by) -> int {
+        if (pr.kmer > 1 && pr.segments > 1)
+            HIP_TRY(ctx, swg_launch_pair_bound_kmer_seg(T.d_tok, T.d_pair_off, b, en, pr.kmer, (uint32_t)pr.segments, ctx->prune_colmax, ctx->kmer_first[pr.kmer - 4].d,
+                                                        ctx->kmer_first[pr.kmer - 4].bits, gated_by, L.bounds, L.ids, qs));
+        else if (pr.kmer > 1)
+            HIP_TRY(ctx, swg_launch_pair_bound_kmer(T.d_tok, T.d_pair_off, en, pr.kmer, ctx->prune_colmax, ctx->kmer_first[pr.kmer - 4].d,
                                                     ctx->kmer_first[pr.kmer - 4].bits, L.bounds, L.ids, qs));
-    else if (pr.kmer > 1)
-        HIP_TRY(ctx, swg_launch_pair_bound_kmer(T.d_tok, T.d_pair_off, n_pairs, pr.kmer, ctx->prune_colmax, ctx->kmer_first[pr.kmer - 4].d,
-                                                ctx->kmer_first[pr.kmer - 4].bits, L.bounds, L.ids, qs));
-    else
-        HIP_TRY(ctx, swg_launch_pair_bound(T.d_tok, T.d_pair_off, n_pairs, ctx->prune_colmax, L.bounds, L.ids, qs));
-    if (pr.fixed) HIP_TRY(ctx, hipMemsetD32Async(reinterpret_cast<hipDeviceptr_t>(thr), (int)pr.fixed_T, 1, qs));
+        else
+            HIP_TRY(ctx, swg_launch_pair_bound(T.d_tok, T.d_pair_off, en, ctx->prune_colmax, L.bounds, L.ids, qs));
+        return SWG_OK;
+    };
+    const SwgPruneBoundRange br = swg_prune_bound_range(stages, n_pairs);
+    if (br.stage == stages.size()) {
+        const int rc = first_level(br.begin, br.end, nullptr);
+        if (rc != SWG_OK) return rc;
+    } else if (br.skip_end > br.skip_begin)
+        HIP_TRY(ctx, hipMemsetD32Async(reinterpret_cast<hipDeviceptr_t>(L.bounds + br.skip_begin), (int)SWG_PRUNE_NOT_BOUNDED, br.skip_end - br.skip_begin, qs));
     db->prune_stages.clear();
-    for (const SwgPruneStage &st : swg_prune_stages(pr, F->segs)) {
+    for (const SwgPruneStage &st : stages) {
         if (st.queued & SWG_STAGE_THRESHOLD)
             HIP_TRY(ctx, swg_launch_prune_threshold(db->d_scores, db->d_order, (uint32_t)((size_t)db->n_bins * SWG_BIN), (uint32_t)k, db->d_hist, thr, qs));
+        if (st.queued & SWG_STAGE_BOUND) {
+            const int rc = first_level(br.begin, br.end, thr);
+            if (rc != SWG_OK) return rc;
+        }
         if (st.queued & SWG_STAGE_PREFIX_CUT) HIP_TRY(ctx, swg_launch_prune_cut(L.bounds, T.d_pair_off, st.begin, st.end, thr, cut_word, qs));
         if (st.queued & SWG_STAGE_GATE) HIP_TRY(ctx, swg_launch_prune_refine_gate(L.bounds, st.begin, st.end, thr, gate, qs));
         if (st.queued & SWG_STAGE_REFINE)
@@ -2082,7 +2100,9 @@
     P->prune.refine4 = P->prune.prefix_cut || ctx->kmer_fourth_refused
                            ? 0
                            : swg_prune_refine4_choice(ka, P->prune.kmer, P->prune.segments, P->prune.refine, P->prune.refine3);
-    ctx->prune_choice = SwgPruneChoice{P->prune.kmer, P->prune.segments, P->prune.refine, P->prune.refine3, P->prune.refine4};
+    ka.forced_gate = ctx->opt_prune_gate;
+    P->prune.gate = !P->prune.prefix_cut && swg_prune_gate_choice(ka, P->prune.kmer, P->prune.segments);
+    ctx->prune_choice = SwgPruneChoice{P->prune.kmer, P->prune.segments, P->prune.refine, P->prune.refine3, P->prune.refine4, P->prune.gate ? 1 : 0};
     return SWG_OK;
 }
 
@@ -2647,6 +2667,12 @@
     out[1] = (int64_t)ctx->kmer_refine4_builds;
     out[2] = ctx->kmer_fourth.d && ctx->kmer_fourth.epoch == ctx->epoch ? ctx->kmer_fourth.bits : 0;
     out[3] = ctx->kmer_fourth_refused ? 1 : 0;
+    return SWG_OK;
+}
+extern "C" int swg_debug_prune_gate(swg_ctx *ctx, int64_t *out)
+{
+    if (!ctx || !out) return swg_set_ctx_error(ctx, SWG_ERR_ARG, "swg_debug_prune_gate: NULL argument");
+    out[0] = ctx->prune_choice.gate;
     return SWG_OK;
 }
 extern "C" int swg_debug_prune_refine4_read(swg_ctx *ctx, const uint32_t *blocks, size_t n, uint16_t *out)
diff --git a/seq-align-gpu_amd/csrc/swg_diag_host.cpp b/seq-align-gpu_amd/csrc/swg_diag_host.cpp
--- a/seq-align-gpu_amd/csrc/swg_diag_host.cpp
+++ b/seq-align-gpu_amd/csrc/swg_diag_host.cpp
@@ -560,6 +560,7 @@
     for (size_t si = 0; si < stages.size(); ++si) {
         if (si == 0 && !plan.fixed) continue;
         uint32_t q = plan.fixed ? 0u : SWG_STAGE_THRESHOLD;
+        if (plan.gate && si == (plan.fixed ? 0u : 1u)) q |= SWG_STAGE_BOUND;
         if (plan.prefix_cut) q |= SWG_STAGE_PREFIX_CUT;
         else {
             if (plan.refine && plan.fixed && si == 0 && stages.size() > 1) q |= SWG_STAGE_GATE;
@@ -573,6 +574,13 @@
     return stages;
 }
 
+SwgPruneBoundRange swg_prune_bound_range(const std::vector<SwgPruneStage> &stages, uint32_t n_pairs)
+{
+    for (size_t i = 0; i < stages.size(); ++i)
+        if (stages[i].queued & SWG_STAGE_BOUND) return SwgPruneBoundRange{i, stages[i].begin, stages.back().end, stages.front().begin, stages[i].begin};
+    return SwgPruneBoundRange{stages.size(), 0u, n_pairs, 0u, 0u};
+}
+
 static int debug_prune_stages(const int64_t *in, int head, int64_t *out, size_t cap, size_t *n_out)
 {
     if (!in || !n_out || (cap > 0 && !out) || in[0] < 0 || in[head - 1] < 0) return SWG_ERR_ARG;
@@ -580,7 +588,8 @@
     plan.on = true;
     plan.head_pairs = (uint32_t)in[0], plan.fixed = in[1] != 0, plan.refine = (int)in[2], plan.prefix_cut = in[3] != 0;
     plan.refine3 = head >= 6 ? (int)in[4] : 0;
-    plan.refine4 = head == 7 ? (int)in[5] : 0;
+    plan.refine4 = head >= 7 ? (int)in[5] : 0;
+    plan.gate = head == 8 && in[6] != 0;
     std::vector<std::pair<uint32_t, uint32_t>> segments;
     for (int64_t i = 0; i < in[head - 1]; ++i) segments.emplace_back((uint32_t)in[head + 2 * i], (uint32_t)in[head + 1 + 2 * i]);
     const std::vector<SwgPruneStage> stages = swg_prune_stages(plan, segments);
@@ -592,6 +601,7 @@
 extern "C" int swg_debug_prune_stages(const int64_t *in, int64_t *out, size_t cap, size_t *n_out) { return debug_prune_stages(in, 5, out, cap, n_out); }
 extern "C" int swg_debug_prune_stages3(const int64_t *in, int64_t *out, size_t cap, size_t *n_out) { return debug_prune_stages(in, 6, out, cap, n_out); }
 extern "C" int swg_debug_prune_stages4(const int64_t *in, int64_t *out, size_t cap, size_t *n_out) { return debug_prune_stages(in, 7, out, cap, n_out); }
+extern "C" int swg_debug_prune_stages5(const int64_t *in, int64_t *out, size_t cap, size_t *n_out) { return debug_prune_stages(in, 8, out, cap, n_out); }
 
 void swg_kmer_cprof(const int8_t *rows, const int8_t *idx, size_t lq, int8_t *cprof)
 {
@@ -878,16 +888,41 @@
 
 #define SWG_REFINE3_GAIN 0.0151
 #define SWG_REFINE3_BOUND_ROW 1.74e-12
+static bool refine3_pays(const SwgKmerAsk &a)
+{
+    if (a.table_rate <= 0 || a.fill_rate <= 0 || a.lq == 0) return false;
+    const double cost = (double)swg_kmer_entries(4) * 4 * (double)a.lq / a.table_rate + SWG_REFINE3_BOUND_ROW * (double)a.pair_rows;
+    const double gain = SWG_REFINE3_GAIN * (double)a.pair_rows / a.fill_rate;
+    return cost <= 0.5 * gain;
+}
 int swg_prune_refine3_choice(const SwgKmerAsk &a, int k, int S, int S2)
 {
     if (!a.pruned || k < 1) return 0;
     if (a.forced_refine3 == 256) return 256;
     if (a.forced_refine3 != 0 || a.forced != 0 || a.forced_segments != 0 || a.forced_refine != 0) return 0;
     if (k != 4 || S <= 1 || S2 != 128 || a.table_bits != 8) return 0;
-    if (a.table_rate <= 0 || a.fill_rate <= 0 || a.lq == 0) return 0;
-    const double cost = (double)swg_kmer_entries(4) * 4 * (double)a.lq / a.table_rate + SWG_REFINE3_BOUND_ROW * (double)a.pair_rows;
-    const double gain = SWG_REFINE3_GAIN * (double)a.pair_rows / a.fill_rate;
-    return cost <= 0.5 * gain ? 256 : 0;
+    return refine3_pays(a) ? 256 : 0;
+}
+
+bool swg_prune_gate_choice(const SwgKmerAsk &a, int k, int S)
+{
+    if (!a.pruned || k <= 1 || S <= 1 || a.forced_gate == 1) return false;
+    if (a.forced_gate == 2) return true;
+    if (a.forced != 0 || a.forced_segments != 0) return false;
+    return refine3_pays(a);
+}
+
+extern "C" int swg_debug_prune_gate_choice(const int64_t *in, int64_t *out)
+{
+    SwgKmerAsk a;
+    if (!debug_kmer_ask(in, out, 8, &a)) return SWG_ERR_ARG;
+    if (!swg_prune_gate_value_ok((long)in[8])) return SWG_ERR_ARG;
+    a.forced_gate = (long)in[8];
+    int S = 0;
+    out[0] = swg_prune_kmer_choice(a, &S);
+    out[1] = S;
+    out[2] = swg_prune_gate_choice(a, (int)out[0], S) ? 1 : 0;
+    return SWG_OK;
 }
 
 extern "C" int swg_debug_prune_refine3_choice(const int64_t *in, int64_t *out)
diff --git a/seq-align-gpu_amd/csrc/swg_host_internal.h b/seq-align-gpu_amd/csrc/swg_host_internal.h
--- a/seq-align-gpu_amd/csrc/swg_host_internal.h
+++ b/seq-align-gpu_amd/csrc/swg_host_internal.h
@@ -205,6 +205,7 @@
     int refine3 = 0;
     int refine4 = 0;
     bool prefix_cut = false;
+    bool gate = false;
     bool fixed = false;
     uint32_t fixed_T = 0;
 };
@@ -222,7 +223,7 @@
 SwgPrunePlan swg_prune_plan(const SwgPruneAsk &a);
 enum : uint32_t {
     SWG_STAGE_THRESHOLD = 1u, SWG_STAGE_PREFIX_CUT = 2u, SWG_STAGE_GATE = 4u, SWG_STAGE_REFINE = 8u, SWG_STAGE_LIST = 16u, SWG_STAGE_REFINE3 = 32u,
-    SWG_STAGE_REFINE4 = 64u
+    SWG_STAGE_REFINE4 = 64u, SWG_STAGE_BOUND = 128u
 };
 struct SwgPruneStage {
     uint32_t begin, end;
@@ -230,9 +231,16 @@
     uint32_t queued;
 };
 std::vector<SwgPruneStage> swg_prune_stages(const SwgPrunePlan &plan, const std::vector<std::pair<uint32_t, uint32_t>> &segments);
+#define SWG_PRUNE_NOT_BOUNDED 0xFFFFFFFFu
+struct SwgPruneBoundRange {
+    size_t stage;
+    uint32_t begin, end, skip_begin, skip_end;
+};
+SwgPruneBoundRange swg_prune_bound_range(const std::vector<SwgPruneStage> &stages, uint32_t n_pairs);
 extern "C" int swg_debug_prune_stages(const int64_t *in, int64_t *out, size_t cap, size_t *n_out);
 extern "C" int swg_debug_prune_stages3(const int64_t *in, int64_t *out, size_t cap, size_t *n_out);
 extern "C" int swg_debug_prune_stages4(const int64_t *in, int64_t *out, size_t cap, size_t *n_out);
+extern "C" int swg_debug_prune_stages5(const int64_t *in, int64_t *out, size_t cap, size_t *n_out);
 #define SWG_PRUNE_ABOVE_AUTO_PAIRS 16u
 inline bool swg_prune_above_auto(uint64_t range_pairs, uint64_t groups) { return range_pairs >= SWG_PRUNE_ABOVE_AUTO_PAIRS * std::max<uint64_t>(1, groups); }
 inline int swg_above_multi_route(long option, bool admitted, bool single_pruned)
@@ -262,6 +270,7 @@
     long forced_refine = 0;
     long forced_refine3 = 0;
     long forced_refine4 = 0;
+    long forced_gate = 0;
     int table_bits5 = 8;
     int table_bits = 8;
     bool pruned = false;
@@ -297,6 +306,9 @@
 extern "C" int swg_debug_prune_refine4_choice(const int64_t *in, int64_t *out);
 extern "C" int swg_debug_prune_kmer_refine4(const int8_t *rows, const int8_t *idx, size_t lq, int gap_open, int gap_extend, int S4, const int8_t *flat,
                                             const uint64_t *offsets, size_t n, uint64_t *u_out);
+bool swg_prune_gate_choice(const SwgKmerAsk &a, int k, int S);
+inline bool swg_prune_gate_value_ok(long v) { return v == 0 || v == 1 || v == 2; }
+extern "C" int swg_debug_prune_gate_choice(const int64_t *in, int64_t *out);
 #define SWG_PRUNE_WORD_T 18u
 #define SWG_PRUNE_WORD_CUT 20u
 #define SWG_ABOVE_WORD_COUNT 24u
@@ -368,6 +380,7 @@
 };
 struct SwgPruneChoice {
     int kmer = 0, segments = 0, refine = 0, refine3 = 0, refine4 = 0;
+    int gate = 0;
 };
 
 #define SWG_MAX_INFLIGHT 4
@@ -442,6 +455,7 @@
     long opt_prune_refine = 0;
     long opt_prune_refine3 = 0;
     long opt_prune_refine4 = 0;
+    long opt_prune_gate = 0;
     long opt_prune_table_bits = 0;
     long opt_prune_cut = 0;
     int8_t *d_kmer_cprof = nullptr;
diff --git a/seq-align-gpu_amd/csrc/swg_internal.h b/seq-align-gpu_amd/csrc/swg_internal.h
--- a/seq-align-gpu_amd/csrc/swg_internal.h
+++ b/seq-align-gpu_amd/csrc/swg_internal.h
@@ -245,8 +245,8 @@
                                  int k, uint32_t S, int8_t *d_cprof, void *d_table, int bits, hipStream_t stream);
 hipError_t swg_launch_pair_bound_kmer(const uint4 *d_tok, const uint32_t *d_pair_off, uint32_t n_pairs, int k, const SwgColMax &cm,
                                       const void *d_table, int bits, uint32_t *d_bound, uint32_t *d_ids, hipStream_t stream);
-hipError_t swg_launch_pair_bound_kmer_seg(const uint4 *d_tok, const uint32_t *d_pair_off, uint32_t n_pairs, int k, uint32_t S, const SwgColMax &cm,
-                                          const void *d_table, int bits, uint32_t *d_bound, uint32_t *d_ids, hipStream_t stream);
+hipError_t swg_launch_pair_bound_kmer_seg(const uint4 *d_tok, const uint32_t *d_pair_off, uint32_t begin, uint32_t end, int k, uint32_t S, const SwgColMax &cm,
+                                          const void *d_table, int bits, const uint32_t *d_thr, uint32_t *d_bound, uint32_t *d_ids, hipStream_t stream);
 hipError_t swg_launch_prune_threshold(const int32_t *d_scores, const uint32_t *d_order, uint32_t n_slots, uint32_t k, uint32_t *d_hist,
                                       uint32_t *d_thr, hipStream_t stream);
 hipError_t swg_launch_prune_cut(const uint32_t *d_bound, const uint32_t *d_pair_off, uint32_t begin, uint32_t end, const uint32_t *d_thr,
diff --git a/seq-align-gpu_amd/csrc/swg_kernels.hip b/seq-align-gpu_amd/csrc/swg_kernels.hip
--- a/seq-align-gpu_amd/csrc/swg_kernels.hip
+++ b/seq-align-gpu_amd/csrc/swg_kernels.hip
@@ -2720,20 +2720,43 @@
     }
 }
 
-template <int K, int WD, class E>
-__global__ __launch_bounds__(256) void swg_pair_bound_kmer_seg_kernel(const uint4 *tok, const uint32_t *pair_off, uint32_t n_pairs, SwgColMax cm,
-                                                                      const E *table, uint32_t S, uint32_t *bound, uint32_t *ids)
+template <int K, int WD, class E, bool GATED>
+__device__ __forceinline__ void swg_pair_bound_kmer_seg_body(const uint4 *tok, const uint32_t *pair_off, uint32_t begin, uint32_t n_pairs, const SwgColMax &cm,
+                                                             const E *table, uint32_t S, const uint32_t *thr, uint32_t *bound, uint32_t *ids)
 {
     __shared__ uint32_t lut[32];
     if (threadIdx.x < 32u) lut[threadIdx.x] = swg_kmer_class(threadIdx.x) | (uint32_t)cm.v[threadIdx.x] << 8;
     __syncthreads();
-    const uint32_t p = blockIdx.x * (256u / WD) + threadIdx.x / WD, l = threadIdx.x & (WD - 1u);
+    const uint32_t p = (GATED ? begin : 0u) + blockIdx.x * (256u / WD) + threadIdx.x / WD, l = threadIdx.x & (WD - 1u);
     const uint32_t C = SWG_KMER_CLASSES;
     const bool has = l < S;
     const E *tl = table + (has ? l : 0u);
     const uint32_t m1 = (l & 7u) >= 1u ? 0xFFFFFFFFu : 0u, m2 = (l & 7u) >= 2u ? 0xFFFFFFFFu : 0u, m4 = (l & 7u) >= 4u ? 0xFFFFFFFFu : 0u;
     uint32_t hx = 0u, hy = 0u;
-    if (p < n_pairs) {
+    bool walk = p < n_pairs;
+    if (GATED && walk) {
+        const uint32_t e = pair_off[p + 1u];
+        uint32_t sx = 0u, sy = 0u;
+        for (uint32_t b = pair_off[p] + l; b < e; b += WD) {
+            const uint4 k = tok[b];
+            sx += (lut[(k.x >> 3) & 31u] >> 8) + (lut[(k.y >> 3) & 31u] >> 8) + (lut[(k.z >> 3) & 31u] >> 8) + (lut[(k.w >> 3) & 31u] >> 8);
+            sy += (lut[(k.x >> 11) & 31u] >> 8) + (lut[(k.y >> 11) & 31u] >> 8) + (lut[(k.z >> 11) & 31u] >> 8) + (lut[(k.w >> 11) & 31u] >> 8);
+        }
+#pragma unroll
+        for (int d = WD / 2; d >= 1; d >>= 1) {
+            sx += (uint32_t)__shfl_xor((int)sx, d, WD);
+            sy += (uint32_t)__shfl_xor((int)sy, d, WD);
+        }
+        const uint32_t u1 = sx > sy ? sx : sy;
+        if (u1 < thr[0]) {
+            if (l == WD - 1u) {
+                bound[p] = u1;
+                ids[p] = p;
+            }
+            walk = false;
+        }
+    }
+    if (walk) {
         const uint32_t b0 = pair_off[p], e = pair_off[p + 1u];
         uint32_t tail = b0;
         if (K == 5) {
@@ -2778,39 +2801,65 @@
         }
     }
     const uint32_t h = hx > hy ? hx : hy, u = swg_seg_prefix_max<WD>(h, m1, m2, m4);
-    if (p < n_pairs && l == WD - 1u) {
+    if ((GATED ? walk : p < n_pairs) && l == WD - 1u) {
         bound[p] = u;
         ids[p] = p;
     }
 }
 
+template <int K, int WD, class E>
+__global__ __launch_bounds__(256) void swg_pair_bound_kmer_seg_kernel(const uint4 *tok, const uint32_t *pair_off, uint32_t n_pairs, SwgColMax cm,
+                                                                      const E *table, uint32_t S, uint32_t *bound, uint32_t *ids)
+{
+    swg_pair_bound_kmer_seg_body<K, WD, E, false>(tok, pair_off, 0u, n_pairs, cm, table, S, nullptr, bound, ids);
+}
+
+template <int K, int WD, class E>
+__global__ __launch_bounds__(256) void swg_pair_bound_kmer_seg_gated_kernel(const uint4 *tok, const uint32_t *pair_off, uint32_t begin, uint32_t end,
+                                                                            SwgColMax cm, const E *table, uint32_t S, const uint32_t *thr, uint32_t *bound,
+                                                                            uint32_t *ids)
+{
+    swg_pair_bound_kmer_seg_body<K, WD, E, true>(tok, pair_off, begin, end, cm, table, S, thr, bound, ids);
+}
+
 template <int K, class E>
-static void swg_launch_pair_bound_kmer_seg_k(const uint4 *d_tok, const uint32_t *d_pair_off, uint32_t n_pairs, const SwgColMax &cm,
-                                             const E *d_table, uint32_t S, uint32_t *d_bound, uint32_t *d_ids, hipStream_t stream)
-{
+static void swg_launch_pair_bound_kmer_seg_k(const uint4 *d_tok, const uint32_t *d_pair_off, uint32_t begin, uint32_t end, const SwgColMax &cm,
+                                             const E *d_table, uint32_t S, const uint32_t *d_thr, uint32_t *d_bound, uint32_t *d_ids, hipStream_t stream)
+{
+    const uint32_t n = end - begin;
+    if (d_thr) {
+        if (S <= 8u)
+            hipLaunchKernelGGL((swg_pair_bound_kmer_seg_gated_kernel<K, 8, E>), dim3((n + 31u) / 32u), dim3(256), 0, stream, d_tok, d_pair_off, begin, end, cm, d_table, S, d_thr, d_bound, d_ids);
+        else if (S <= 16u)
+            hipLaunchKernelGGL((swg_pair_bound_kmer_seg_gated_kernel<K, 16, E>), dim3((n + 15u) / 16u), dim3(256), 0, stream, d_tok, d_pair_off, begin, end, cm, d_table, S, d_thr, d_bound, d_ids);
+        else
+            hipLaunchKernelGGL((swg_pair_bound_kmer_seg_gated_kernel<K, 32, E>), dim3((n + 7u) / 8u), dim3(256), 0, stream, d_tok, d_pair_off, begin, end, cm, d_table, S, d_thr, d_bound, d_ids);
+        return;
+    }
     if (S <= 8u)
-        hipLaunchKernelGGL((swg_pair_bound_kmer_seg_kernel<K, 8, E>), dim3((n_pairs + 31u) / 32u), dim3(256), 0, stream, d_tok, d_pair_off, n_pairs, cm, d_table, S, d_bound, d_ids);
+        hipLaunchKernelGGL((swg_pair_bound_kmer_seg_kernel<K, 8, E>), dim3((n + 31u) / 32u), dim3(256), 0, stream, d_tok, d_pair_off, n, cm, d_table, S, d_bound, d_ids);
     else if (S <= 16u)
-        hipLaunchKernelGGL((swg_pair_bound_kmer_seg_kernel<K, 16, E>), dim3((n_pairs + 15u) / 16u), dim3(256), 0, stream, d_tok, d_pair_off, n_pairs, cm, d_table, S, d_bound, d_ids);
+        hipLaunchKernelGGL((swg_pair_bound_kmer_seg_kernel<K, 16, E>), dim3((n + 15u) / 16u), dim3(256), 0, stream, d_tok, d_pair_off, n, cm, d_table, S, d_bound, d_ids);
     else
-        hipLaunchKernelGGL((swg_pair_bound_kmer_seg_kernel<K, 32, E>), dim3((n_pairs + 7u) / 8u), dim3(256), 0, stream, d_tok, d_pair_off, n_pairs, cm, d_table, S, d_bound, d_ids);
-}
-
-hipError_t swg_launch_pair_bound_kmer_seg(const uint4 *d_tok, const uint32_t *d_pair_off, uint32_t n_pairs, int k, uint32_t S, const SwgColMax &cm,
-                                          const void *d_table, int bits, uint32_t *d_bound, uint32_t *d_ids, hipStream_t stream)
-{
-    if ((k != 4 && k != 5) || S == 0u || S > SWG_KMER_MAX_SEGMENTS || (bits != 8 && bits != 16)) return hipErrorInvalidValue;
-    if (n_pairs == 0) return hipSuccess;
+        hipLaunchKernelGGL((swg_pair_bound_kmer_seg_kernel<K, 32, E>), dim3((n + 7u) / 8u), dim3(256), 0, stream, d_tok, d_pair_off, n, cm, d_table, S, d_bound, d_ids);
+}
+
+hipError_t swg_launch_pair_bound_kmer_seg(const uint4 *d_tok, const uint32_t *d_pair_off, uint32_t begin, uint32_t end, int k, uint32_t S, const SwgColMax &cm,
+                                          const void *d_table, int bits, const uint32_t *d_thr, uint32_t *d_bound, uint32_t *d_ids, hipStream_t stream)
+{
+    if ((k != 4 && k != 5) || S == 0u || S > SWG_KMER_MAX_SEGMENTS || (bits != 8 && bits != 16) || end < begin || (!d_thr && begin != 0u))
+        return hipErrorInvalidValue;
+    if (end == begin) return hipSuccess;
     const uint8_t *t8 = static_cast<const uint8_t *>(d_table);
     const uint16_t *t16 = static_cast<const uint16_t *>(d_table);
     if (k == 5 && bits == 8)
-        swg_launch_pair_bound_kmer_seg_k<5>(d_tok, d_pair_off, n_pairs, cm, t8, S, d_bound, d_ids, stream);
+        swg_launch_pair_bound_kmer_seg_k<5>(d_tok, d_pair_off, begin, end, cm, t8, S, d_thr, d_bound, d_ids, stream);
     else if (k == 5)
-        swg_launch_pair_bound_kmer_seg_k<5>(d_tok, d_pair_off, n_pairs, cm, t16, S, d_bound, d_ids, stream);
+        swg_launch_pair_bound_kmer_seg_k<5>(d_tok, d_pair_off, begin, end, cm, t16, S, d_thr, d_bound, d_ids, stream);
     else if (bits == 8)
-        swg_launch_pair_bound_kmer_seg_k<4>(d_tok, d_pair_off, n_pairs, cm, t8, S, d_bound, d_ids, stream);
+        swg_launch_pair_bound_kmer_seg_k<4>(d_tok, d_pair_off, begin, end, cm, t8, S, d_thr, d_bound, d_ids, stream);
     else
-        swg_launch_pair_bound_kmer_seg_k<4>(d_tok, d_pair_off, n_pairs, cm, t16, S, d_bound, d_ids, stream);
+        swg_launch_pair_bound_kmer_seg_k<4>(d_tok, d_pair_off, begin, end, cm, t16, S, d_thr, d_bound, d_ids, stream);
     return hipGetLastError();
 }
 
```

New measurement: 49910 (median of 6 runs). 1.02x the previous value.
